# MichSchli/RelationPrediction

Measured on AMD Instinct MI355X. Metric: processed edges/sec (R-GCN forward+backward), FB15k-237 gcn_block, higher is better.
Workload: dtype f32 (dense contractions: fp32 operands split exactly into 3 bf16, 6 of 9 partial products on the bf16 matrix cores, fp32 accumulation; error vs float64 equal to the fp32 MFMA's); 1 GPU; fb237_block; entities=14541, relations=237, dim=500, layers=2, kind=block, num_blocks_or_bases=100, graph_edges=15000, norm_mode=intended (1/deg of the edge's own row; SURVEY H1, DESIGN section 10), parallelism=single GPU

## Files before the change

### include/rgcn_devtools.h

```cpp
#ifndef RGCN_DEVTOOLS_H_
#define RGCN_DEVTOOLS_H_

#include "rgcn.h"

#ifdef __cplusplus
extern "C" {
#endif
#if defined(__GNUC__)
#pragma GCC visibility push(default)
#endif

rgcn_status rgcn_debug_gemm(rgcn_ctx* ctx, int32_t trans_a, int32_t trans_b, int32_t M, int32_t N,
                            int32_t K, int32_t split_k, const float* a_host, const float* b_host,
                            float* c_host);

rgcn_status rgcn_debug_gemm_time(rgcn_ctx* ctx, int32_t trans_a, int32_t trans_b, int32_t M, int32_t N,
                                 int32_t K, int32_t split_k, int32_t iters, const float* a_host,
                                 const float* b_host, float* avg_ms);

rgcn_status rgcn_debug_gemm_presplit(rgcn_ctx* ctx, int32_t trans_b, int32_t M, int32_t N, int32_t K, int32_t iters,
                                     const float* a_host, const float* b_host, float* c_host, float* avg_ms);

rgcn_status rgcn_debug_xcd_map(rgcn_ctx* ctx, int32_t n_blocks, int32_t* out_host);

#if defined(__GNUC__)
#pragma GCC visibility pop
#endif
#ifdef __cplusplus
}
#endif
#endif
```

### relationprediction_amd/_native.py

```python
from __future__ import annotations

import ctypes as C
import os

import numpy as np

_HERE = os.path.dirname(os.path.abspath(__file__))
LIB_PATH = os.path.join(_HERE, "lib", "librgcn.so")

ABI_VERSION = 1
KIND_BLOCK, KIND_BASIS = 0, 1
NORM_INTENDED, NORM_TF_AS_EXECUTED, NORM_NONE, NORM_LOCAL = 0, 1, 2, 3
BUF_EXCHANGE, BUF_SELF, BUF_DSELF_EXCHANGE, BUF_INDEG, BUF_OUTDEG, BUF_ROWPTR, BUF_NORM_EXCHANGE, \
    BUF_DBASIS_EXCHANGE, BUF_PERM_VERTEX, BUF_PERM_RELATION, BUF_RANK_ENERGIES, BUF_MSG_NORM = range(12)

KINDS = {"block": KIND_BLOCK, "basis": KIND_BASIS}
NORMS = {"intended": NORM_INTENDED, "tf_as_executed": NORM_TF_AS_EXECUTED, "none": NORM_NONE, "local": NORM_LOCAL}

INPUT_EMBEDDING, INPUT_ONEHOT = 0, 1
INPUT_MODES = {"embedding": INPUT_EMBEDDING, "onehot": INPUT_ONEHOT}


def norm_mode_value(norm_mode):
    if isinstance(norm_mode, str):
        if norm_mode not in NORMS:
            raise ValueError("IncidenceNormalization / norm_mode must be one of %s, not %r"
                             % (", ".join(sorted(NORMS, key=NORMS.get)), norm_mode))
        return NORMS[norm_mode]
    return int(norm_mode)


class RgcnError(RuntimeError):
    def __init__(self, status, message):
        super().__init__("librgcn status %d: %s" % (status, message))
        self.status = status


class RgcnConfig(C.Structure):
    _fields_ = [
        ("abi_version", C.c_int32), ("device", C.c_int32), ("num_entities", C.c_int32),
        ("num_relations", C.c_int32), ("dim", C.c_int32), ("num_layers", C.c_int32),
        ("kind", C.c_int32), ("num_bases", C.c_int32), ("keep_prob", C.c_float),
        ("norm_mode", C.c_int32), ("max_edges", C.c_int64), ("rank", C.c_int32),
        ("world", C.c_int32), ("input_mode", C.c_int32),
    ]


_lib = None

_P = C.c_void_p
_SIGS = {
    "rgcn_abi_version": (C.c_int32, []),
    "rgcn_create": (C.c_int32, [C.POINTER(RgcnConfig), C.POINTER(_P)]),
    "rgcn_destroy": (C.c_int32, [_P]),
    "rgcn_last_error": (C.c_char_p, [_P]),
    "rgcn_sync": (C.c_int32, [_P]),
    "rgcn_param_count": (C.c_int32, [_P]),
    "rgcn_param_info": (C.c_int32, [_P, C.c_int32, C.c_char_p, C.c_int32, C.POINTER(C.c_int64), C.POINTER(C.c_int32)]),
    "rgcn_set_param": (C.c_int32, [_P, C.c_int32, _P, C.c_int64]),
    "rgcn_get_param": (C.c_int32, [_P, C.c_int32, _P, C.c_int64]),
    "rgcn_get_grad": (C.c_int32, [_P, C.c_int32, _P, C.c_int64]),
    "rgcn_set_graph": (C.c_int32, [_P, _P, C.c_int64]),
    "rgcn_set_graph_device": (C.c_int32, [_P, _P, C.c_int64]),
    "rgcn_forward": (C.c_int32, [_P, C.c_int32, C.c_uint64, _P]),
    "rgcn_get_codes": (C.c_int32, [_P, _P, C.c_int64]),
    "rgcn_get_activation": (C.c_int32, [_P, C.c_int32, _P, C.c_int64]),
    "rgcn_get_dropout_mask": (C.c_int32, [_P, C.c_int32, _P, C.c_int64]),
    "rgcn_codes_device": (_P, [_P]),
    "rgcn_backward": (C.c_int32, [_P, _P, C.c_int64]),
    "rgcn_backward_device": (C.c_int32, [_P, _P]),
    "rgcn_step_device": (C.c_int32, [_P, _P, C.c_int64, C.c_int32, C.c_uint64, _P]),
    "rgcn_decoder_reserve": (C.c_int32, [_P, C.c_int64]),
    "rgcn_decoder_loss_backward_device": (C.c_int32, [_P, _P, _P, C.c_int64, C.c_float]),
    "rgcn_dcodes_device": (_P, [_P]),
    "rgcn_get_loss": (C.c_int32, [_P, C.POINTER(C.c_double)]),
    "rgcn_optimizer_config": (C.c_int32, [_P, C.c_float, C.c_float, C.c_float, C.c_float, C.c_float]),
    "rgcn_sampler_create": (C.c_int32, [_P, C.c_int64, C.c_int32, C.POINTER(_P)]),
    "rgcn_sampler_destroy": (None, [_P]),
    "rgcn_sampler_edge_neighborhood": (C.c_int32, [_P, C.c_int64, C.c_uint64, _P]),
    "rgcn_neighborhood_reserve": (C.c_int32, [_P, _P, C.c_int64]),
    "rgcn_sample_neighborhood_device": (C.c_int32, [_P, C.c_int64, C.c_uint64, _P, C.c_int32]),
    "rgcn_capture_begin": (C.c_int32, [_P]),
    "rgcn_capture_end": (C.c_int32, [_P, C.POINTER(C.c_int32)]),
    "rgcn_graph_launch": (C.c_int32, [_P, C.c_int32]),
    "rgcn_graph_destroy": (C.c_int32, [_P, C.c_int32]),
    "rgcn_negative_sample_device": (C.c_int32, [_P, _P, C.c_int64, C.c_int32, C.c_uint64, _P, _P]),
    "rgcn_rank_reserve": (C.c_int32, [_P, C.c_int64]),
    "rgcn_rank_device": (C.c_int32, [_P, _P, C.c_int64, C.c_int32, _P, _P, _P, _P]),
    "rgcn_topk_device": (C.c_int32, [_P, _P, C.c_int64, C.c_int32, C.c_int32, _P, _P, _P, _P]),
    "rgcn_optimizer_step": (C.c_int32, [_P]),
    "rgcn_optimizer_norm_partial": (C.c_int32, [_P]),
    "rgcn_optimizer_apply": (C.c_int32, [_P]),
    "rgcn_train_step_device": (C.c_int32, [_P, _P, C.c_int64, _P, _P, C.c_int64, C.c_uint64, C.c_float]),
    "rgcn_prefetch_graph_device": (C.c_int32, [_P, _P, C.c_int64]),
    "rgcn_prefetch_graph_dropout_device": (C.c_int32, [_P, _P, C.c_int64, C.c_int64, C.c_uint64]),
    "rgcn_set_graph_dropout_device": (C.c_int32, [_P, _P, C.c_int64, C.c_int64, C.c_uint64, _P]),
    "rgcn_get_graph_edges": (C.c_int32, [_P, _P, C.c_int64]),
    "rgcn_train_step_minibatch_device": (C.c_int32, [_P, _P, C.c_int64, C.c_int64, C.c_uint64, C.c_int32, C.c_uint64,
                                                     _P, _P, C.c_uint64, C.c_float]),
    "rgcn_set_relation_owner": (C.c_int32, [_P, _P, C.c_int32]),
    "rgcn_comm_unique_id": (C.c_int32, [_P]),
    "rgcn_comm_init": (C.c_int32, [_P, _P]),
    "rgcn_comm_allreduce_sum": (C.c_int32, [_P, _P, C.c_int64]),
    "rgcn_forward_begin": (C.c_int32, [_P, C.c_int32, C.c_uint64, _P]),
    "rgcn_forward_layer_partial": (C.c_int32, [_P, C.c_int32]),
    "rgcn_forward_layer_finish": (C.c_int32, [_P, C.c_int32]),
    "rgcn_backward_begin": (C.c_int32, [_P, _P]),
    "rgcn_backward_layer_partial": (C.c_int32, [_P, C.c_int32]),
    "rgcn_backward_layer_finish": (C.c_int32, [_P, C.c_int32]),
    "rgcn_backward_end": (C.c_int32, [_P]),
    "rgcn_read_buffer": (C.c_int32, [_P, C.c_int32, _P, C.c_int64]),
    "rgcn_write_buffer": (C.c_int32, [_P, C.c_int32, _P, C.c_int64]),
    "rgcn_device_alloc": (C.c_int32, [_P, C.c_int64, C.POINTER(_P)]),
    "rgcn_device_free": (C.c_int32, [_P, _P]),
    "rgcn_copy_to_device": (C.c_int32, [_P, _P, _P, C.c_int64]),
    "rgcn_copy_to_device_async": (C.c_int32, [_P, _P, _P, C.c_int64, C.c_int32]),
    "rgcn_copy_to_host": (C.c_int32, [_P, _P, _P, C.c_int64]),
    "rgcn_timer_start": (C.c_int32, [_P]),
    "rgcn_timer_stop": (C.c_int32, [_P, C.POINTER(C.c_float)]),
    "rgcn_set_overlap": (C.c_int32, [_P, C.c_int32]),
    "rgcn_set_gemm_mode": (C.c_int32, [_P, C.c_int32]),
    "rgcn_set_fusion": (C.c_int32, [_P, C.c_int32]),
    "rgcn_comm_info": (C.c_int32, [_P, C.POINTER(C.c_int32), C.POINTER(C.c_int32), C.POINTER(C.c_int32)]),
    "rgcn_device_info": (C.c_int32, [C.c_int32, C.POINTER(C.c_int32), C.POINTER(C.c_int64)]),
    "rgcn_profile_enable": (C.c_int32, [_P, C.c_int32]),
    "rgcn_profile_reset": (C.c_int32, [_P]),
    "rgcn_profile_count": (C.c_int32, [_P]),
    "rgcn_profile_get_compulsory": (C.c_int32, [_P, C.c_int32, C.POINTER(C.c_double)]),
    "rgcn_profile_get": (C.c_int32, [_P, C.c_int32, C.c_char_p, C.c_int32, C.POINTER(C.c_int64),
                                    C.POINTER(C.c_double), C.POINTER(C.c_double), C.POINTER(C.c_double)]),
}
_DEVTOOLS_SIGS = {
    "rgcn_debug_gemm": (C.c_int32, [_P, C.c_int32, C.c_int32, C.c_int32, C.c_int32, C.c_int32, C.c_int32, _P, _P, _P]),
    "rgcn_debug_xcd_map": (C.c_int32, [_P, C.c_int32, _P]),
    "rgcn_debug_gemm_presplit": (C.c_int32, [_P, C.c_int32, C.c_int32, C.c_int32, C.c_int32, C.c_int32, _P, _P, _P,
                                             C.POINTER(C.c_float)]),
    "rgcn_debug_gemm_time": (C.c_int32, [_P, C.c_int32, C.c_int32, C.c_int32, C.c_int32, C.c_int32, C.c_int32,
                                         C.c_int32, _P, _P, C.POINTER(C.c_float)]),
}
_lib_devtools = None


def exported_symbols():
    return sorted(_SIGS)


def exported_devtools_symbols():
    return sorted(_DEVTOOLS_SIGS)


def load_library(path=None, devtools=False):
    global _lib, _lib_devtools
    if devtools:
        if _lib_devtools is None or path is not None:
            p = path or os.path.join(os.path.dirname(LIB_PATH), "librgcn_devtools.so")
            if not os.path.exists(p):
                raise ImportError("%s not found: python -m relationprediction_amd.build makes it" % p)
            lib = C.CDLL(p, mode=C.RTLD_LOCAL)
            for name, (res, args) in list(_SIGS.items()) + list(_DEVTOOLS_SIGS.items()):
                fn = getattr(lib, name)
                fn.restype = res
                fn.argtypes = args
            if path is not None:
                return lib
            _lib_devtools = lib
        return _lib_devtools
    if _lib is not None and path is None:
        return _lib
    if path is None and os.environ.get("RGCN_LIBRARY") == "devtools":
        _lib = load_library(devtools=True)
        return _lib
    p = path or LIB_PATH
    if not os.path.exists(p):
        raise ImportError(
            "%s not found: build the HIP library first (python -m relationprediction_amd.build, or "
            "__graft_entry__.build()).  There is no CPU fallback." % p)
    lib = C.CDLL(p, mode=C.RTLD_GLOBAL)
    for name, (res, args) in _SIGS.items():
        fn = getattr(lib, name)
        fn.restype = res
        fn.argtypes = args
    if lib.rgcn_abi_version() != ABI_VERSION:
        raise ImportError("librgcn.so ABI version %d != binding %d" % (lib.rgcn_abi_version(), ABI_VERSION))
    if path is None:
        _lib = lib
    return lib


def _ptr(a):
    return a.ctypes.data_as(C.c_void_p)


class DeviceBuffer:

    def __init__(self, engine, nbytes):
        self.engine = engine
        self.nbytes = int(nbytes)
        p = C.c_void_p()
        engine._check(engine.lib.rgcn_device_alloc(engine.ctx, self.nbytes, C.byref(p)))
        self.ptr = p

    def upload(self, arr):
        arr = np.ascontiguousarray(arr)
        assert arr.nbytes == self.nbytes, (arr.nbytes, self.nbytes)
        self.engine._check(self.engine.lib.rgcn_copy_to_device(self.engine.ctx, self.ptr, _ptr(arr), arr.nbytes))
        return self

    def download(self, dtype, shape):
        out = np.empty(shape, dtype=dtype)
        assert out.nbytes <= self.nbytes
        self.engine._check(self.engine.lib.rgcn_copy_to_host(self.engine.ctx, _ptr(out), self.ptr, out.nbytes))
        return out

    def free(self):
        if self.ptr is not None and self.engine.ctx is not None:
            self.engine.lib.rgcn_device_free(self.engine.ctx, self.ptr)
        self.ptr = None


class NeighborhoodSampler:

    def __init__(self, triples, num_entities):
        self.lib = load_library()
        t = np.ascontiguousarray(triples, dtype=np.int32).reshape(-1, 3)
        self.n = len(t)
        h = C.c_void_p()
        st = self.lib.rgcn_sampler_create(_ptr(t), self.n, int(num_entities), C.byref(h))
        if st != 0:
            raise RgcnError(st, "rgcn_sampler_create (ids out of range or empty graph)")
        self.handle = h

    def sample(self, sample_size, seed):
        out = np.empty(int(sample_size), dtype=np.int32)
        st = self.lib.rgcn_sampler_edge_neighborhood(self.handle, int(sample_size), C.c_uint64(int(seed)), _ptr(out))
        if st != 0:
            raise RgcnError(st, "rgcn_sampler_edge_neighborhood (sample_size %d of %d edges)" % (sample_size, self.n))
        return out

    def close(self):
        if getattr(self, "handle", None) is not None:
            self.lib.rgcn_sampler_destroy(self.handle)
            self.handle = None

    __del__ = close


class Engine:

    def __init__(self, num_entities, num_relations, dim, num_layers, kind, num_bases, keep_prob=0.8,
                 norm_mode="intended", max_edges=0, device=0, rank=0, world=1, devtools=False, input_mode="embedding"):
        self.lib = load_library(devtools=devtools)
        self.ctx = None
        cfg = RgcnConfig()
        cfg.abi_version = ABI_VERSION
        cfg.device = int(device)
        cfg.num_entities = int(num_entities)
        cfg.num_relations = int(num_relations)
        cfg.dim = int(dim)
        cfg.num_layers = int(num_layers)
        cfg.kind = KINDS[kind] if isinstance(kind, str) else int(kind)
        cfg.num_bases = int(num_bases)
        cfg.keep_prob = float(keep_prob)
        cfg.norm_mode = norm_mode_value(norm_mode)
        cfg.max_edges = int(max_edges)
        cfg.rank = int(rank)
        cfg.world = int(world)
        cfg.input_mode = INPUT_MODES[input_mode] if isinstance(input_mode, str) else int(input_mode)
        self.cfg = cfg
        ctx = C.c_void_p()
        st = self.lib.rgcn_create(C.byref(cfg), C.byref(ctx))
        if st != 0:
            raise RgcnError(st, (self.lib.rgcn_last_error(None) or b"").decode())
        self.ctx = ctx
        self.V, self.R, self.d, self.L = cfg.num_entities, cfg.num_relations, cfg.dim, cfg.num_layers
        self.max_edges = int(cfg.max_edges)
        self.param_names, self.param_shapes = [], []
        for i in range(self.lib.rgcn_param_count(self.ctx)):
            name = C.create_string_buffer(64)
            shape = (C.c_int64 * 4)()
            nd = C.c_int32()
            self._check(self.lib.rgcn_param_info(self.ctx, i, name, 64, shape, C.byref(nd)))
            self.param_names.append(name.value.decode())
            self.param_shapes.append(tuple(int(shape[k]) for k in range(nd.value)))

    def _check(self, st):
        if st != 0:
            raise RgcnError(st, (self.lib.rgcn_last_error(self.ctx) or b"").decode())

    def close(self):
        if self.ctx is not None:
            if getattr(self, "_rank_buf", None) is not None:
                self._rank_buf.free()
                self._rank_buf = None
            self.lib.rgcn_destroy(self.ctx)
            self.ctx = None

    def __del__(self):
        try:
            self.close()
        except Exception:
            pass

    def __enter__(self):
        return self

    def __exit__(self, *a):
        self.close()

    def sync(self):
        self._check(self.lib.rgcn_sync(self.ctx))

    def _index(self, key):
        return key if isinstance(key, int) else self.param_names.index(key)

    def set_param(self, key, value):
        i = self._index(key)
        a = np.ascontiguousarray(value, dtype=np.float32)
        if tuple(a.shape) != self.param_shapes[i]:
            raise ValueError("%s: shape %s != %s" % (self.param_names[i], a.shape, self.param_shapes[i]))
        self._check(self.lib.rgcn_set_param(self.ctx, i, _ptr(a), a.size))

    def set_params(self, params):
        for n in self.param_names:
            self.set_param(n, params[n])

    def get_param(self, key):
        i = self._index(key)
        out = np.empty(self.param_shapes[i], dtype=np.float32)
        self._check(self.lib.rgcn_get_param(self.ctx, i, _ptr(out), out.size))
        return out

    def get_grad(self, key):
        i = self._index(key)
        out = np.empty(self.param_shapes[i], dtype=np.float32)
        self._check(self.lib.rgcn_get_grad(self.ctx, i, _ptr(out), out.size))
        return out

    def get_grads(self):
        return {n: self.get_grad(n) for n in self.param_names}

    def get_params(self):
        return {n: self.get_param(n) for n in self.param_names}

    def set_graph(self, triples):
        t = np.asarray(triples)
        if t.size == 0:
            t = np.zeros((0, 3), dtype=np.int32)
        if t.ndim != 2 or t.shape[1] != 3:
            raise ValueError("graph_edges must be [E,3]")
        if t.dtype != np.int32:
            if t.size and (t.min() < -2 ** 31 or t.max() >= 2 ** 31):
                raise ValueError("ids do not fit int32")
            t = t.astype(np.int32)
        t = np.ascontiguousarray(t)
        self._check(self.lib.rgcn_set_graph(self.ctx, _ptr(t), t.shape[0]))
        self.num_edges = int(t.shape[0])

    def set_graph_device(self, dev_buffer, num_edges):
        self._check(self.lib.rgcn_set_graph_device(self.ctx, dev_buffer.ptr, int(num_edges)))
        self.num_edges = int(num_edges)

    def set_graph_dropout_device(self, batch_buffer, num_edges, keep, seed=0, keep_mask=None):
        self._check(self.lib.rgcn_set_graph_dropout_device(self.ctx, batch_buffer.ptr, int(num_edges), int(keep),
                                                           C.c_uint64(seed), keep_mask.ptr if keep_mask else None))
        self.num_edges = int(keep)

    def graph_edges(self):
        out = np.empty((self.num_edges, 3), dtype=np.int32)
        self._check(self.lib.rgcn_get_graph_edges(self.ctx, _ptr(out), self.num_edges))
        return out

    def prefetch_graph_dropout_device(self, batch_buffer, num_edges, keep, seed):
        self._check(self.lib.rgcn_prefetch_graph_dropout_device(self.ctx, batch_buffer.ptr, int(num_edges), int(keep),
                                                                C.c_uint64(seed)))

    def train_step_minibatch_device(self, batch_buffer, num_edges, keep, edge_seed, rate, negative_seed, x_dev, y_dev,
                                    seed=0, reg_param=0.01):
        self._check(self.lib.rgcn_train_step_minibatch_device(
            self.ctx, batch_buffer.ptr, int(num_edges), int(keep), C.c_uint64(edge_seed), int(rate),
            C.c_uint64(negative_seed), x_dev.ptr, y_dev.ptr, C.c_uint64(seed), C.c_float(reg_param)))
        self.num_edges = int(keep)

    def set_relation_owner(self, owner):
        o = np.ascontiguousarray(owner, dtype=np.int32)
        self._check(self.lib.rgcn_set_relation_owner(self.ctx, _ptr(o), o.size))

    def _masks(self, masks):
        if masks is None:
            return None, None
        m = np.ascontiguousarray(np.stack([np.asarray(x) for x in masks]).astype(np.uint8))
        if m.shape != (self.L, self.V, self.d):
            raise ValueError("dropout masks must be [L,V,d]")
        return m, _ptr(m)

    def forward(self, train=True, seed=0, masks=None):
        m, p = self._masks(masks)
        self._check(self.lib.rgcn_forward(self.ctx, 1 if train else 0, C.c_uint64(seed), p))

    def codes(self):
        return self.activation(self.L)

    def activation(self, layer):
        out = np.empty((self.V, self.d), dtype=np.float32)
        self._check(self.lib.rgcn_get_activation(self.ctx, int(layer), _ptr(out), out.size))
        return out

    def dropout_mask(self, layer):
        out = np.empty((self.V, self.d), dtype=np.uint8)
        self._check(self.lib.rgcn_get_dropout_mask(self.ctx, int(layer), _ptr(out), out.size))
        return out

    def backward(self, dcodes):
        g = np.ascontiguousarray(dcodes, dtype=np.float32)
        if g.shape != (self.V, self.d):
            raise ValueError("dcodes must be [V,d]")
        self._check(self.lib.rgcn_backward(self.ctx, _ptr(g), g.size))

    def backward_device(self, dev_buffer):
        self._check(self.lib.rgcn_backward_device(self.ctx, dev_buffer.ptr))

    def step_device(self, triples_dev, num_edges, dcodes_dev, train=True, seed=0):
        self._check(self.lib.rgcn_step_device(self.ctx, triples_dev.ptr, int(num_edges), 1 if train else 0,
                                              C.c_uint64(seed), dcodes_dev.ptr))
        self.num_edges = int(num_edges)

    def decoder_reserve(self, max_triples):
        self._check(self.lib.rgcn_decoder_reserve(self.ctx, int(max_triples)))

    def decoder_loss_backward_device(self, x_dev, y_dev, num_triples, reg_param):
        self._check(self.lib.rgcn_decoder_loss_backward_device(self.ctx, x_dev.ptr, y_dev.ptr, int(num_triples),
                                                               C.c_float(reg_param)))

    def backward_from_decoder(self):
        self._check(self.lib.rgcn_backward_device(self.ctx, self.lib.rgcn_dcodes_device(self.ctx)))

    def dcodes(self):
        out = np.empty((self.V, self.d), dtype=np.float32)
        self._check(self.lib.rgcn_copy_to_host(self.ctx, _ptr(out), self.lib.rgcn_dcodes_device(self.ctx), out.nbytes))
        return out

    def loss(self):
        v = C.c_double()
        self._check(self.lib.rgcn_get_loss(self.ctx, C.byref(v)))
        return float(v.value)

    def capture_begin(self):
        self._check(self.lib.rgcn_capture_begin(self.ctx))

    def capture_end(self):
        gid = C.c_int32(-1)
        self._check(self.lib.rgcn_capture_end(self.ctx, C.byref(gid)))
        return int(gid.value)

    def graph_launch(self, graph_id):
        self._check(self.lib.rgcn_graph_launch(self.ctx, int(graph_id)))

    def graph_destroy(self, graph_id):
        self._check(self.lib.rgcn_graph_destroy(self.ctx, int(graph_id)))

    def neighborhood_reserve(self, train_triples):
        t = np.ascontiguousarray(train_triples, dtype=np.int32).reshape(-1, 3)
        self._check(self.lib.rgcn_neighborhood_reserve(self.ctx, _ptr(t), len(t)))
        self._nbr_edges = len(t)

    def sample_neighborhood_device(self, sample_size, seed, batch_dev, on_prefetch_stream=False):
        self._check(self.lib.rgcn_sample_neighborhood_device(self.ctx, int(sample_size), C.c_uint64(int(seed)),
                                                             batch_dev.ptr, 1 if on_prefetch_stream else 0))

    def negative_sample_device(self, batch_dev, n, rate, seed, x_dev, y_dev):
        self._check(self.lib.rgcn_negative_sample_device(self.ctx, batch_dev.ptr, int(n), int(rate), C.c_uint64(int(seed)),
                                                         x_dev.ptr, y_dev.ptr))

    def rank_reserve(self, max_queries):
        self._check(self.lib.rgcn_rank_reserve(self.ctx, int(max_queries)))
        self._rank_reserved = max(getattr(self, "_rank_reserved", 0), int(max_queries))

    def ranks(self, triples, predict_object, filter_ptr, filter_idx):
        x = np.ascontiguousarray(triples, dtype=np.int32).reshape(-1, 3)
        n = len(x)
        if n == 0:
            return np.zeros(0, np.int32), np.zeros(0, np.int32)
        fp = np.ascontiguousarray(filter_ptr, dtype=np.int64)
        fi = np.ascontiguousarray(filter_idx, dtype=np.int32)
        assert fp.shape == (n + 1,) and fp[-1] == len(fi)
        nnz = max(len(fi), 1)
        off_x, off_fi = 8 * (n + 1), 8 * (n + 1) + 12 * n
        off_out = (off_fi + 4 * nnz + 7) // 8 * 8
        total = off_out + 8 * n
        if getattr(self, "_rank_buf", None) is None or self._rank_buf.nbytes < total:
            if getattr(self, "_rank_buf", None) is not None:
                self._rank_buf.free()
            self._rank_buf = DeviceBuffer(self, max(total, 1 << 20))
        base = self._rank_buf.ptr.value if hasattr(self._rank_buf.ptr, "value") else int(self._rank_buf.ptr)
        head = np.empty(off_fi, dtype=np.uint8)
        head[:off_x] = fp.view(np.uint8)
        head[off_x:] = x.reshape(-1).view(np.uint8)
        self._check(self.lib.rgcn_copy_to_device_async(self.ctx, C.c_void_p(base), _ptr(head), off_fi, 0))
        fb = fi.view(np.uint8)
        for lo in range(0, len(fb), 1 << 20):
            part = fb[lo:lo + (1 << 20)]
            self._check(self.lib.rgcn_copy_to_device_async(self.ctx, C.c_void_p(base + off_fi + lo), _ptr(part), len(part), 0))
        self._check(self.lib.rgcn_rank_device(self.ctx, C.c_void_p(base + off_x), n, 1 if predict_object else 0,
                                              C.c_void_p(base), C.c_void_p(base + off_fi), C.c_void_p(base + off_out),
                                              C.c_void_p(base + off_out + 4 * n)))
        out = np.empty(2 * n, dtype=np.int32)
        self._check(self.lib.rgcn_copy_to_host(self.ctx, _ptr(out), C.c_void_p(base + off_out), 8 * n))
        return out[:n].copy(), out[n:].copy()

    def topk(self, queries, predict_object, k, exclude_ptr=None, exclude_idx=None):
        x = np.ascontiguousarray(queries, dtype=np.int32).reshape(-1, 3)
        n, k = len(x), int(k)
        if (exclude_ptr is None) != (exclude_idx is None):
            raise ValueError("exclude_ptr and exclude_idx come together")
        if n == 0:
            return np.zeros((0, max(k, 0)), np.int32), np.zeros((0, max(k, 0)), np.float32)
        has = exclude_ptr is not None
        fp = np.ascontiguousarray(exclude_ptr if has else np.zeros(n + 1), dtype=np.int64)
        fi = np.ascontiguousarray(exclude_idx if has else np.zeros(0), dtype=np.int32)
        assert fp.shape == (n + 1,) and fp[-1] == len(fi)
        nnz = max(len(fi), 1)
        off_x, off_fi = 8 * (n + 1), 8 * (n + 1) + 12 * n
        off_out = (off_fi + 4 * nnz + 7) // 8 * 8
        room = min(max(k, 0), 1024)
        total = off_out + 8 * n * room
        if getattr(self, "_rank_buf", None) is None or self._rank_buf.nbytes < total:
            if getattr(self, "_rank_buf", None) is not None:
                self._rank_buf.free()
            self._rank_buf = DeviceBuffer(self, max(total, 1 << 20))
        base = self._rank_buf.ptr.value if hasattr(self._rank_buf.ptr, "value") else int(self._rank_buf.ptr)
        head = np.empty(off_fi, dtype=np.uint8)
        head[:off_x] = fp.view(np.uint8)
        head[off_x:] = x.reshape(-1).view(np.uint8)
        for lo in range(0, off_fi, 1 << 20):
            part = head[lo:lo + (1 << 20)]
            self._check(self.lib.rgcn_copy_to_device_async(self.ctx, C.c_void_p(base + lo), _ptr(part), len(part), 0))
        fb = fi.view(np.uint8)
        for lo in range(0, len(fb), 1 << 20):
            part = fb[lo:lo + (1 << 20)]
            self._check(self.lib.rgcn_copy_to_device_async(self.ctx, C.c_void_p(base + off_fi + lo), _ptr(part), len(part), 0))
        self._check(self.lib.rgcn_topk_device(self.ctx, C.c_void_p(base + off_x), n, 1 if predict_object else 0, k,
                                              C.c_void_p(base) if has else None,
                                              C.c_void_p(base + off_fi) if has else None, C.c_void_p(base + off_out),
                                              C.c_void_p(base + off_out + 4 * n * k)))
        out = np.empty(2 * n * k, dtype=np.int32)
        self._check(self.lib.rgcn_copy_to_host(self.ctx, _ptr(out), C.c_void_p(base + off_out), 8 * n * k))
        return out[:n * k].reshape(n, k).copy(), out[n * k:].view(np.float32).reshape(n, k).copy()

    def optimizer_config(self, lr=0.01, beta1=0.9, beta2=0.999, eps=1e-8, max_grad_norm=1.0):
        self._check(self.lib.rgcn_optimizer_config(self.ctx, lr, beta1, beta2, eps, max_grad_norm))

    def optimizer_step(self):
        self._check(self.lib.rgcn_optimizer_step(self.ctx))

    def optimizer_norm_partial(self):
        self._check(self.lib.rgcn_optimizer_norm_partial(self.ctx))

    def optimizer_apply(self):
        self._check(self.lib.rgcn_optimizer_apply(self.ctx))

    def train_step_device(self, triples_dev, num_edges, x_dev, y_dev, num_triples, seed=0, reg_param=0.01):
        self._check(self.lib.rgcn_train_step_device(self.ctx, triples_dev.ptr, int(num_edges), x_dev.ptr, y_dev.ptr,
                                                    int(num_triples), C.c_uint64(seed), C.c_float(reg_param)))
        self.num_edges = int(num_edges)

    def prefetch_graph_device(self, triples_dev, num_edges):
        self._check(self.lib.rgcn_prefetch_graph_device(self.ctx, triples_dev.ptr, int(num_edges)))

    def forward_begin(self, train=True, seed=0, masks=None):
        m, p = self._masks(masks)
        self._check(self.lib.rgcn_forward_begin(self.ctx, 1 if train else 0, C.c_uint64(seed), p))

    def forward_layer_partial(self, l):
        self._check(self.lib.rgcn_forward_layer_partial(self.ctx, l))

    def forward_layer_finish(self, l):
        self._check(self.lib.rgcn_forward_layer_finish(self.ctx, l))

    def backward_begin(self, dcodes_dev=None):
        ptr = self.lib.rgcn_dcodes_device(self.ctx) if dcodes_dev is None else dcodes_dev.ptr
        self._check(self.lib.rgcn_backward_begin(self.ctx, ptr))

    def backward_layer_partial(self, l):
        self._check(self.lib.rgcn_backward_layer_partial(self.ctx, l))

    def backward_layer_finish(self, l):
        self._check(self.lib.rgcn_backward_layer_finish(self.ctx, l))

    def backward_end(self):
        self._check(self.lib.rgcn_backward_end(self.ctx))

    def read_buffer(self, which):
        if which in (BUF_INDEG, BUF_OUTDEG):
            out = np.empty(self.V, dtype=np.int32)
        elif which == BUF_ROWPTR:
            out = np.empty(self.V + 1, dtype=np.int32)
        elif which in (BUF_PERM_VERTEX, BUF_PERM_RELATION):
            out = np.empty(2 * self.num_edges, dtype=np.int32)
        elif which == BUF_MSG_NORM:
            out = np.empty(2 * self.num_edges, dtype=np.float32)
        elif which == BUF_RANK_ENERGIES:
            out = np.empty((getattr(self, "_rank_reserved", 0), self.V), dtype=np.float32)
        elif which == BUF_DSELF_EXCHANGE:
            out = np.empty((self.d, self.d), dtype=np.float32)
        elif which == BUF_NORM_EXCHANGE:
            out = np.empty(1, dtype=np.float32)
        elif which == BUF_DBASIS_EXCHANGE:
            out = np.empty((2, int(self.cfg.num_bases), self.d, self.d), dtype=np.float32)
        else:
            out = np.empty((self.V, self.d), dtype=np.float32)
        self._check(self.lib.rgcn_read_buffer(self.ctx, which, _ptr(out), out.nbytes))
        return out

    def write_buffer(self, which, arr):
        a = np.ascontiguousarray(arr, dtype=np.float32)
        self._check(self.lib.rgcn_write_buffer(self.ctx, which, _ptr(a), a.nbytes))

    @staticmethod
    def comm_unique_id():
        lib = load_library()
        buf = (C.c_uint8 * 128)()
        st = lib.rgcn_comm_unique_id(buf)
        if st != 0:
            raise RgcnError(st, (lib.rgcn_last_error(None) or b"").decode())
        return bytes(buf)

    @staticmethod
    def device_info(device=0):
        lib = load_library()
        n, pci = C.c_int32(0), C.c_int64(-1)
        st = lib.rgcn_device_info(int(device), C.byref(n), C.byref(pci))
        if st != 0:
            raise RgcnError(st, (lib.rgcn_last_error(None) or b"").decode())
        return n.value, pci.value

    def comm_init(self, unique_id):
        buf = (C.c_uint8 * 128).from_buffer_copy(bytes(unique_id))
        self._check(self.lib.rgcn_comm_init(self.ctx, buf))

    def comm_info(self):
        n, r, dev = C.c_int32(-1), C.c_int32(-1), C.c_int32(-1)
        self._check(self.lib.rgcn_comm_info(self.ctx, C.byref(n), C.byref(r), C.byref(dev)))
        return n.value, r.value, dev.value

    def comm_allreduce_sum(self, dev_buffer, count):
        self._check(self.lib.rgcn_comm_allreduce_sum(self.ctx, dev_buffer.ptr, int(count)))

    def alloc(self, nbytes):
        return DeviceBuffer(self, nbytes)

    def copy_to_device(self, buf, arr):
        arr = np.ascontiguousarray(arr)
        assert arr.nbytes <= buf.nbytes
        self._check(self.lib.rgcn_copy_to_device(self.ctx, buf.ptr, _ptr(arr), arr.nbytes))

    def copy_to_device_async(self, buf, arr, on_prefetch_stream=False):
        arr = np.ascontiguousarray(arr)
        assert arr.nbytes <= buf.nbytes
        self._check(self.lib.rgcn_copy_to_device_async(self.ctx, buf.ptr, _ptr(arr), arr.nbytes,
                                                       1 if on_prefetch_stream else 0))

    def to_device(self, arr):
        arr = np.ascontiguousarray(arr)
        return DeviceBuffer(self, arr.nbytes).upload(arr)

    def timer_start(self):
        self._check(self.lib.rgcn_timer_start(self.ctx))

    def timer_stop(self):
        ms = C.c_float()
        self._check(self.lib.rgcn_timer_stop(self.ctx, C.byref(ms)))
        return float(ms.value)

    def set_overlap(self, on=True):
        self._check(self.lib.rgcn_set_overlap(self.ctx, 1 if on else 0))

    def set_fusion(self, mode):
        self._check(self.lib.rgcn_set_fusion(self.ctx, int(mode)))

    def set_gemm_mode(self, mode):
        self._check(self.lib.rgcn_set_gemm_mode(self.ctx, int(mode)))

    def profile_enable(self, on=True):
        self._check(self.lib.rgcn_profile_enable(self.ctx, 1 if on else 0))

    def profile_reset(self):
        self._check(self.lib.rgcn_profile_reset(self.ctx))

    def profile(self):
        out = []
        n = self.lib.rgcn_profile_count(self.ctx)
        for i in range(n):
            name = C.create_string_buffer(64)
            calls = C.c_int64()
            ms, by, fl = C.c_double(), C.c_double(), C.c_double()
            self._check(self.lib.rgcn_profile_get(self.ctx, i, name, 64, C.byref(calls), C.byref(ms),
                                                  C.byref(by), C.byref(fl)))
            cb = C.c_double()
            self._check(self.lib.rgcn_profile_get_compulsory(self.ctx, i, C.byref(cb)))
            out.append({"name": name.value.decode(), "calls": calls.value, "total_ms": ms.value,
                        "alg_bytes": by.value, "alg_flops": fl.value, "compulsory_bytes": cb.value})
        return out

    def debug_gemm_presplit(self, a, b, trans_b=False, iters=0):
        a = np.ascontiguousarray(a, dtype=np.float32)
        b = np.ascontiguousarray(b, dtype=np.float32)
        M, K = a.shape
        N = b.shape[0] if trans_b else b.shape[1]
        out = np.empty((M, N), dtype=np.float32)
        ms = C.c_float()
        self._check(self.lib.rgcn_debug_gemm_presplit(self.ctx, int(trans_b), M, N, K, int(iters), _ptr(a), _ptr(b),
                                                      _ptr(out), C.byref(ms)))
        return (out, float(ms.value)) if iters else out

    def debug_xcd_map(self, n_blocks):
        out = np.zeros(int(n_blocks), dtype=np.int32)
        self._check(self.lib.rgcn_debug_xcd_map(self.ctx, int(n_blocks), _ptr(out)))
        return out

    def debug_gemm_time(self, a, b, trans_a=False, trans_b=False, split_k=0, iters=20):
        a = np.ascontiguousarray(a, dtype=np.float32)
        b = np.ascontiguousarray(b, dtype=np.float32)
        K, M = (a.shape if trans_a else a.shape[::-1])
        N = b.shape[0] if trans_b else b.shape[1]
        ms = C.c_float()
        self._check(self.lib.rgcn_debug_gemm_time(self.ctx, int(trans_a), int(trans_b), M, N, K, int(split_k),
                                                  int(iters), _ptr(a), _ptr(b), C.byref(ms)))
        return float(ms.value)

    def debug_gemm(self, a, b, trans_a=False, trans_b=False, split_k=0):
        a = np.ascontiguousarray(a, dtype=np.float32)
        b = np.ascontiguousarray(b, dtype=np.float32)
        K, M = (a.shape if trans_a else a.shape[::-1])
        N = b.shape[0] if trans_b else b.shape[1]
        assert (b.shape[1] if trans_b else b.shape[0]) == K
        out = np.empty((M, N), dtype=np.float32)
        self._check(self.lib.rgcn_debug_gemm(self.ctx, int(trans_a), int(trans_b), M, N, K, int(split_k),
                                             _ptr(a), _ptr(b), _ptr(out)))
        return out
```

### relationprediction_amd/build.py

```python
from __future__ import annotations

import hashlib
import os
import shutil
import subprocess
import sys
from concurrent.futures import ThreadPoolExecutor

HERE = os.path.dirname(os.path.abspath(__file__))
ROOT = os.path.dirname(HERE)
CSRC = os.path.join(HERE, "csrc")
OBJDIR = os.path.join(ROOT, "build", "obj")
LIBDIR = os.path.join(HERE, "lib")
LIB = os.path.join(LIBDIR, "librgcn.so")
LIB_DEVTOOLS = os.path.join(LIBDIR, "librgcn_devtools.so")
ARCH = "gfx950"
SOURCES = ["rgcn_api.hip", "rgcn_schedule.hip", "rgcn_devtools.hip", "graph_prep.hip", "csr_sort.hip", "gemm_f32.hip", "gemm_bf16x3.hip", "gemm_bf16x3_w8.hip", "block_msgs.hip", "block_rows.hip", "basis.hip", "basis_onehot.hip",
           "elementwise.hip", "decoder.hip", "optimizer.hip", "ranking.hip", "sampler.hip", "neighborhood.hip", "comm.hip"]
HEADERS = [os.path.join(CSRC, "rgcn_internal.h"), os.path.join(CSRC, "rgcn_api_internal.h"), os.path.join(CSRC, "gemm_split.h"), os.path.join(ROOT, "include", "rgcn.h"),
           os.path.join(ROOT, "include", "rgcn_devtools.h")]
DEVTOOLS_SOURCES = ["rgcn_api.hip", "rgcn_devtools.hip", "comm.hip", "decoder.hip", "gemm_bf16x3.hip", "gemm_bf16x3_w8.hip"]
NO_PACKED_FP32 = ["-Xclang", "-target-feature", "-Xclang", "-packed-fp32-ops"]
FLAGS = ["--offload-arch=" + ARCH, "-O3", "-std=c++17", "-fPIC", "-fvisibility=hidden", "-Wall",
         "-Wno-unused-function"] + NO_PACKED_FP32


def _hipcc():
    for cand in (shutil.which("hipcc"), "/opt/rocm/bin/hipcc"):
        if cand and os.path.exists(cand):
            return cand
    raise RuntimeError("hipcc not found: the R-GCN HIP library cannot be built")


def _digest(paths):
    h = hashlib.sha256()
    h.update(" ".join(FLAGS).encode())
    for p in paths:
        with open(p, "rb") as f:
            h.update(f.read())
    return h.hexdigest()


def _llvm_objdump():
    for cand in ("/opt/rocm/lib/llvm/bin/llvm-objdump", shutil.which("llvm-objdump")):
        if cand and os.path.exists(cand):
            return cand
    return None


def check_no_packed_fp32(lib=None):
    import glob
    import re
    import tempfile
    lib = lib or LIB
    objdump = _llvm_objdump()
    if objdump is None:
        raise RuntimeError("llvm-objdump not found: cannot verify the library is free of packed-FP32 ops")
    with tempfile.TemporaryDirectory() as tmp:
        copy = os.path.join(tmp, "lib.so")
        shutil.copy(lib, copy)
        subprocess.run([objdump, "--offloading", copy], capture_output=True, text=True, cwd=tmp, check=True)
        bad = []
        objs = glob.glob(copy + ".*amdgcn*")
        if not objs:
            raise RuntimeError("no device code objects found in " + lib)
        for co in objs:
            r = subprocess.run([objdump, "-d", co], capture_output=True, text=True, check=True)
            bad += re.findall(r"v_pk_(?:fma|mul|add)_f32", r.stdout)
        if bad:
            raise RuntimeError("librgcn.so contains %d packed-FP32 instructions (%s): they are unsafe beside the "
                               "bf16-split GEMM" % (len(bad), ", ".join(sorted(set(bad)))))
    return True


def build(force=False, verbose=False):
    os.makedirs(OBJDIR, exist_ok=True)
    os.makedirs(LIBDIR, exist_ok=True)
    hipcc = _hipcc()
    jobs = []
    for src in SOURCES + [d + "@devtools" for d in DEVTOOLS_SOURCES]:
        dev = src.endswith("@devtools")
        src = src.replace("@devtools", "")
        sp = os.path.join(CSRC, src)
        obj = os.path.join(OBJDIR, src.replace(".hip", ".devtools.o" if dev else ".o"))
        stamp = obj + ".sha"
        dig = _digest([sp] + HEADERS) + ("+devtools" if dev else "")
        fresh = (not force and os.path.exists(obj) and os.path.exists(stamp)
                 and open(stamp).read() == dig)
        jobs.append((sp, obj, stamp, dig, fresh, dev))

    def compile_one(job):
        sp, obj, stamp, dig, fresh, dev = job
        if fresh:
            return None
        cmd = [hipcc] + FLAGS + (["-DRGCN_DEVTOOLS"] if dev else []) + ["-c", sp, "-o", obj]
        r = subprocess.run(cmd, capture_output=True, text=True)
        if r.returncode != 0:
            raise RuntimeError("hipcc failed for %s:\n%s" % (sp, r.stderr[-4000:]))
        with open(stamp, "w") as f:
            f.write(dig)
        return r.stderr if verbose else None

    with ThreadPoolExecutor(max_workers=min(8, len(jobs))) as ex:
        outs = list(ex.map(compile_one, jobs))
    for o in outs:
        if o:
            sys.stderr.write(o)
    product = [j for j in jobs if not j[5]]
    devobj = {os.path.basename(j[0]): j[1] for j in jobs if j[5]}
    stale = any(not j[4] for j in jobs)
    for lib, objs in ((LIB, [j[1] for j in product]),
                      (LIB_DEVTOOLS, [devobj.get(os.path.basename(j[0]), j[1]) for j in product])):
        if force or stale or not os.path.exists(lib):
            vs = os.path.join(OBJDIR, "exports.map")
            with open(vs, "w") as f:
                f.write("{ global: rgcn_*; local: *; };\n")
            cmd = [hipcc, "--offload-arch=" + ARCH, "-shared", "-fPIC", "-Wl,--version-script=" + vs, "-o", lib] + objs + ["-ldl"]
            r = subprocess.run(cmd, capture_output=True, text=True)
            if r.returncode != 0:
                raise RuntimeError("link failed:\n" + r.stderr[-4000:])
            check_no_packed_fp32(lib)
    return LIB


def build_test_collective(force=False, device_side=False):
    root = os.path.dirname(os.path.dirname(os.path.abspath(__file__)))
    name = "ipc_collective" if device_side else "shm_collective"
    src = os.path.join(root, "tests", "collective_double", name + ".hip")
    outdir = os.path.join(root, "tests", "collective_double", "_build")
    out = os.path.join(outdir, "lib%s.so" % name.replace("_", ""))
    stamp = out + ".sha"
    dig = _digest([src])
    if not force and os.path.exists(out) and os.path.exists(stamp) and open(stamp).read() == dig:
        return out
    os.makedirs(outdir, exist_ok=True)
    r = subprocess.run([_hipcc(), "--offload-arch=" + ARCH, "-O2", "-std=c++17", "-fPIC", "-shared", src, "-o", out,
                        "-lrt"], capture_output=True, text=True)
    if r.returncode != 0:
        raise RuntimeError("hipcc failed for %s:\n%s" % (src, r.stderr[-4000:]))
    with open(stamp, "w") as f:
        f.write(dig)
    return out


if __name__ == "__main__":
    print(build(force="--force" in sys.argv, verbose="--verbose" in sys.argv))
```

### relationprediction_amd/csrc/gemm_bf16x3.hip

```cpp
#include <cstdlib>

#include "gemm_split.h"

namespace rgcn {

using namespace gx;

namespace {

template <bool VEC>
__device__ __forceinline__ void load_kc(const float* __restrict__ X, const float* __restrict__ zeros,
                                        int ld, int rows, int row0, int k0, int kend, f32x4 (&r)[2]) {
#pragma unroll
  for (int p = 0; p < 2; ++p) {
    const int f = threadIdx.x + NTH * p;
    const int row = row0 + (f >> 2), k = k0 + (f & 3) * 4;
    const size_t off = (size_t)row * ld + k;
    if constexpr (VEC) {
      const float* src = (row < rows && k < kend) ? X + off : zeros;
      r[p] = *reinterpret_cast<const f32x4*>(src);
    } else {
      float e[4];
#pragma unroll
      for (int q = 0; q < 4; ++q) {
        const float* src = (row < rows && k + q < kend) ? X + off + q : zeros;
        e[q] = *src;
      }
      r[p] = f32x4{e[0], e[1], e[2], e[3]};
    }
  }
}
template <bool VEC>
__device__ __forceinline__ void load_rc(const float* __restrict__ X, const float* __restrict__ zeros,
                                        int ld, int rows, int row0, int k0, int kend, f32x4 (&r)[2]) {
  const int kp = threadIdx.x >> 5, rg = threadIdx.x & 31;
#pragma unroll
  for (int q = 0; q < 2; ++q) {
    const int k = k0 + 2 * kp + q, row = row0 + 4 * rg;
    const size_t off = (size_t)k * ld + row;
    if constexpr (VEC) {
      const float* src = (k < kend && row < rows) ? X + off : zeros;
      r[q] = *reinterpret_cast<const f32x4*>(src);
    } else {
      float e[4];
#pragma unroll
      for (int i = 0; i < 4; ++i) {
        const float* src = (k < kend && row + i < rows) ? X + off + i : zeros;
        e[i] = *src;
      }
      r[q] = f32x4{e[0], e[1], e[2], e[3]};
    }
  }
}

struct SplitRegs {
  u32x4 w;
};
template <bool KC, int PLANE, int C>
__device__ __forceinline__ void split_chunk(f32x4 (&r)[2], SplitRegs& st, uint32_t* __restrict__ lds,
                                            uint32_t negmask) {
  if constexpr (KC) {
    constexpr int q = C / 6, c = C % 6;
    const int f = threadIdx.x + NTH * q;
    uint32_t* dst = lds + (f >> 2) * KC_LD + (f & 3) * 2;
    f32x4& v = r[q];
    if constexpr (c == 0 || c == 2) st.w[0] = split_level<0, 1>(v, v, c == 0 ? negmask : 0u);
    if constexpr (c == 1 || c == 3) {
      st.w[1] = split_level<2, 3>(v, v, c == 1 ? negmask : 0u);
      *reinterpret_cast<uint2*>(dst + (c / 2) * PLANE) = make_uint2(st.w[0], st.w[1]);
    }
    if constexpr (c == 4)
      *reinterpret_cast<uint2*>(dst + 2 * PLANE) = make_uint2(split_last(v[0], v[1]), split_last(v[2], v[3]));
  } else {
    const int kp = threadIdx.x >> 5, rg = threadIdx.x & 31;
    uint32_t* dst = lds + kp * RC_LD + 4 * rg;
    f32x4& e = r[0];
    f32x4& o = r[1];
    if constexpr (C < 8) {
      constexpr int i = C % 4;
      st.w[i] = split_level<i, i>(e, o, C < 4 ? negmask : 0u);
      if constexpr (i == 3) *reinterpret_cast<u32x4*>(dst + (C / 4) * PLANE) = st.w;
    }
    if constexpr (C == 8) { st.w[0] = split_last(e[0], o[0]); st.w[1] = split_last(e[1], o[1]); }
    if constexpr (C == 9) {
      st.w[2] = split_last(e[2], o[2]); st.w[3] = split_last(e[3], o[3]);
      *reinterpret_cast<u32x4*>(dst + 2 * PLANE) = st.w;
    }
  }
}
template <bool KC, int PLANE, int C0, int C1>
__device__ __forceinline__ void split_chunks(f32x4 (&r)[2], SplitRegs& st, uint32_t* __restrict__ lds,
                                             uint32_t negmask = 0u) {
  if constexpr (C0 < C1) {
    split_chunk<KC, PLANE, C0>(r, st, lds, negmask);
    split_chunks<KC, PLANE, C0 + 1, C1>(r, st, lds, negmask);
  }
}

template <bool KC>
__device__ __forceinline__ bf16x8 load_frag(const uint32_t* __restrict__ plane, int row, int h) {
  u32x4 v;
  if constexpr (KC) {
    v = *reinterpret_cast<const u32x4*>(plane + row * KC_LD + 4 * h);
  } else {
    const uint32_t* p = plane + (4 * h) * RC_LD + row;
    v[0] = p[0]; v[1] = p[RC_LD]; v[2] = p[2 * RC_LD]; v[3] = p[3 * RC_LD];
  }
  return __builtin_bit_cast(bf16x8, v);
}

template <bool A_KC, bool B_KC, bool VEC, int TERMS, bool B_PRE = false>
__global__ void __launch_bounds__(NTH, 2) k_gemm_bf16x3(XArgs g) {
  constexpr int PA = A_KC ? KC_PLANE : RC_PLANE, PB = B_KC ? KC_PLANE : RC_PLANE;
  constexpr int TA = 3 * PA, TB = B_PRE ? 0 : 3 * PB;
  extern __shared__ __attribute__((aligned(16))) uint32_t lds[];

  int wg = blockIdx.x;
  const int total = g.tiles_m * g.tiles_n * g.splits;
  if (g.swizzle == 1) {
    const int xcd = wg & 7, idx = wg >> 3;
    const int q = total >> 3, r = total & 7;
    wg = (xcd < r ? xcd * (q + 1) : r * (q + 1) + (xcd - r) * q) + idx;
  }
  const int per_split = g.tiles_m * g.tiles_n;
  int z = wg / per_split;
  const int rem = wg - z * per_split;
  int m0 = (rem / g.tiles_n) * BM, n0 = (rem % g.tiles_n) * BN;
  if (g.swizzle == 2) {
    const int xcd = blockIdx.x & 7, idx = blockIdx.x >> 3;
    const int rp = (idx / g.tiles_n) * 8 + xcd;
    if (rp >= g.tiles_m) return;
    z = 0;
    m0 = rp * BM;
    n0 = (idx % g.tiles_n) * BN;
  }
  const int grp = blockIdx.y;
  int Mlim = g.M, Klim = g.K, kps = g.k_per_split;
  if (g.batch.limit != nullptr) {
    const int n = g.batch.limit[grp * g.batch.limit_stride];
    if (g.batch.limit_on_k) {
      Klim = min(Klim, max(n, 0));
      const int per = (Klim + g.splits - 1) / g.splits;
      kps = max(BK, ((per + BK - 1) / BK) * BK);
    } else {
      Mlim = min(Mlim, n);
      if (m0 >= Mlim) return;
    }
  }
  const float* const gA = g.A + (size_t)grp * g.batch.strideA;
  const float* const gB = g.B + (size_t)grp * g.batch.strideB;
  const int ks = z * kps;
  const int ke = max(ks, min(Klim, ks + kps));
  const int nkt = (ke - ks + BK - 1) / BK;

  const int lane = threadIdx.x & 63, wave = threadIdx.x >> 6;
  const int wm = (wave >> 1) * 64, wn = (wave & 1) * 64;
  const int li = lane & 31, h = lane >> 5;

  f32x16 acc[2][2];
#pragma unroll
  for (int i = 0; i < 2; ++i)
#pragma unroll
    for (int j = 0; j < 2; ++j)
#pragma unroll
      for (int r = 0; r < 16; ++r) acc[i][j][r] = 0.0f;

  f32x4 ra[2][2], rb[2][2];
  auto gload = [&](int k0, f32x4 (&xa)[2], f32x4 (&xb)[2]) {
    if constexpr (A_KC) load_kc<VEC>(gA, g.zeros, g.lda, Mlim, m0, k0, ke, xa);
    else load_rc<VEC>(gA, g.zeros, g.lda, Mlim, m0, k0, ke, xa);
    if constexpr (!B_PRE) {
      if constexpr (B_KC) load_kc<VEC>(gB, g.zeros, g.ldb, g.N, n0, k0, ke, xb);
      else load_rc<VEC>(gB, g.zeros, g.ldb, g.N, n0, k0, ke, xb);
    }
  };
  const float* wa[2];
  const float* wb[2];
  int ia[2] = {0, 0}, ib[2] = {0, 0};
  if constexpr (VEC) {
#pragma unroll
    for (int p = 0; p < 2; ++p) {
      if constexpr (A_KC) {
        const int f = threadIdx.x + NTH * p, row = m0 + (f >> 2);
        wa[p] = row < Mlim ? gA + (size_t)row * g.lda + ks + (f & 3) * 4 : g.zeros;
        ia[p] = row < Mlim ? BK : 0;
      } else {
        const int row = m0 + 4 * (threadIdx.x & 31), k = ks + 2 * (threadIdx.x >> 5) + p;
        wa[p] = row < Mlim ? gA + (size_t)k * g.lda + row : g.zeros;
        ia[p] = row < Mlim ? BK * g.lda : 0;
      }
      if constexpr (B_PRE) {
        wb[p] = g.zeros;
      } else if constexpr (B_KC) {
        const int f = threadIdx.x + NTH * p, row = n0 + (f >> 2);
        wb[p] = row < g.N ? gB + (size_t)row * g.ldb + ks + (f & 3) * 4 : g.zeros;
        ib[p] = row < g.N ? BK : 0;
      } else {
        const int row = n0 + 4 * (threadIdx.x & 31), k = ks + 2 * (threadIdx.x >> 5) + p;
        wb[p] = row < g.N ? gB + (size_t)k * g.ldb + row : g.zeros;
        ib[p] = row < g.N ? BK * g.ldb : 0;
      }
    }
#pragma unroll
    for (int p = 0; p < 2; ++p) { wa[p] += 2 * (size_t)ia[p]; wb[p] += 2 * (size_t)ib[p]; }
  }
  auto gwalk = [&](f32x4 (&xa)[2], f32x4 (&xb)[2]) {
#pragma unroll
    for (int p = 0; p < 2; ++p) {
      xa[p] = *reinterpret_cast<const f32x4*>(wa[p]);
      wa[p] += ia[p];
      if constexpr (!B_PRE) {
        xb[p] = *reinterpret_cast<const f32x4*>(wb[p]);
        wb[p] += ib[p];
      }
    }
  };
  auto sstore = [&](uint32_t* buf, f32x4 (&xa)[2], f32x4 (&xb)[2]) {
    SplitRegs st;
    split_chunks<A_KC, PA, 0, 12>(xa, st, buf);
    if constexpr (!B_PRE) split_chunks<B_KC, PB, 0, 12>(xb, st, buf + TA);
  };
  const int nkt_all = (g.K + BK - 1) / BK;
  const u32x4* const bq = B_PRE ? g.bfrag + (size_t)grp * g.batch.strideBfrag +
                                      ((size_t)((n0 + wn) >> 5) * 6 + h) * 32 + li
                                : nullptr;
  bf16x8 fbp[2][2][3];
  auto bfetch = [&](int kt_abs, bf16x8 (&f)[2][3]) {
    const u32x4* q = bq + (size_t)min(kt_abs, nkt_all - 1) * g.nt32 * 192;
#pragma unroll
    for (int j = 0; j < 2; ++j)
#pragma unroll
      for (int pl = 0; pl < 3; ++pl) f[j][pl] = __builtin_bit_cast(bf16x8, q[(j * 3 + pl) * 64]);
  };
  int flip[3] = {1 << 30, 1 << 30, 1 << 30};
  if (nkt >= 16) {
    flip[0] = max(2, (int)(0.173f * nkt + 0.5f) & ~1);
    flip[1] = (nkt / 2 + 1) & ~1;
    flip[2] = (int)(0.849f * nkt + 0.5f) & ~1;
  }
  auto sign_group = [&](int t) { return (t >= flip[0] ? 1 : 0) + (t >= flip[1] ? 1 : 0) + (t >= flip[2] ? 1 : 0); };
  auto negate_acc = [&]() {
#pragma unroll
    for (int i = 0; i < 2; ++i)
#pragma unroll
      for (int j = 0; j < 2; ++j)
#pragma unroll
        for (int r = 0; r < 16; ++r) acc[i][j][r] = 0.0f - acc[i][j][r];
  };
  auto step = [&](int kt, auto parity, auto walk) {
    constexpr int P = decltype(parity)::value;
    constexpr bool WALK = decltype(walk)::value;
    if (kt == flip[0] || kt == flip[1] || kt == flip[2]) negate_acc();
    const uint32_t negmask = (sign_group(kt + 1) & 1) ? 0x80000000u : 0u;
    if constexpr (WALK) gwalk(ra[P], rb[P]); else gload(ks + (kt + 2) * BK, ra[P], rb[P]);
    if constexpr (B_PRE) bfetch(kt + 1, fbp[1 - P]);
    const uint32_t* a_lds = lds + P * (TA + TB);
    const uint32_t* b_lds = a_lds + TA;
    uint32_t* nxt = lds + (1 - P) * (TA + TB);
    bf16x8 fa[2][3], fb[2][3];
#pragma unroll
    for (int i = 0; i < 2; ++i)
#pragma unroll
      for (int pl = 0; pl < 3; ++pl) fa[i][pl] = load_frag<A_KC>(a_lds + pl * PA, wm + 32 * i + li, h);
#pragma unroll
    for (int j = 0; j < 2; ++j)
#pragma unroll
      for (int pl = 0; pl < 3; ++pl) {
        if constexpr (B_PRE) fb[j][pl] = fbp[P][j][pl];
        else fb[j][pl] = load_frag<B_KC>(b_lds + pl * PB, wn + 32 * j + li, h);
      }
    __builtin_amdgcn_sched_barrier(0);
    constexpr int NP = 9;
    constexpr int pa_[NP] = {2, 2, 1, 2, 0, 1, 1, 0, 0};
    constexpr int pb_[NP] = {2, 1, 2, 0, 2, 1, 0, 1, 0};
    constexpr int NM = 4 * TERMS;
    constexpr int NCH = B_PRE ? 12 : 24;
    constexpr int PER = (NCH + NM - 1) / NM;
    SplitRegs st;
    auto weave = [&](auto mi) {
      constexpr int m = decltype(mi)::value;
      constexpr int t = NP - TERMS + m / 4, i = (m / 2) % 2, j = m % 2;
      acc[i][j] = __builtin_amdgcn_mfma_f32_32x32x16_bf16(fa[i][pa_[t]], fb[j][pb_[t]], acc[i][j], 0, 0, 0);
      constexpr int c0 = B_PRE ? (m % 2 == 0 ? m / 2 : 12) : (m * PER < 24 ? m * PER : 24);
      constexpr int c1 = B_PRE ? (m % 2 == 0 ? (m / 2 + 1 < 12 ? m / 2 + 1 : 12) : 12) : ((m + 1) * PER < 24 ? (m + 1) * PER : 24);
      split_chunks<A_KC, PA, (c0 < 12 ? c0 : 12), (c1 < 12 ? c1 : 12)>(ra[1 - P], st, nxt, negmask);
      if constexpr (!B_PRE)
        split_chunks<B_KC, PB, (c0 > 12 ? c0 - 12 : 0), (c1 > 12 ? c1 - 12 : 0)>(rb[1 - P], st, nxt + TA);
      __builtin_amdgcn_sched_barrier(0);
    };
    static_for<0, NM>(weave);
    lds_barrier();
  };

  if (nkt > 0) {
    gload(ks, ra[0], rb[0]);
    if constexpr (B_PRE) bfetch(0, fbp[0]);
    sstore(lds, ra[0], rb[0]);
    gload(ks + BK, ra[1], rb[1]);
  }
  lds_barrier();
  using I0 = std::integral_constant<int, 0>;
  using I1 = std::integral_constant<int, 1>;
  int kt = 0;
  if constexpr (VEC) {
    const int nwalk = ((ke - ks) / BK - 2) & ~1;
    for (; kt < nwalk; kt += 2) {
      step(kt, I0{}, std::true_type{});
      step(kt + 1, I1{}, std::true_type{});
    }
  }
  for (; kt < nkt; kt += 2) {
    step(kt, I0{}, std::false_type{});
    if (kt + 1 < nkt) step(kt + 1, I1{}, std::false_type{});
  }
  if (nkt > 0 && (sign_group(nkt - 1) & 1)) negate_acc();

  float* C = g.C + (size_t)grp * g.batch.strideC + (size_t)z * g.M * g.ldc;
  if (g.vecC) {
    float* stage = reinterpret_cast<float*>(lds);
#pragma unroll
    for (int pass = 0; pass < 2; ++pass) {
      if (wm == 64 * pass) {
#pragma unroll
        for (int i = 0; i < 2; ++i)
#pragma unroll
          for (int j = 0; j < 2; ++j)
#pragma unroll
            for (int r = 0; r < 16; ++r) {
              const int row = 32 * i + (r & 3) + 8 * (r >> 2) + 4 * h;
              stage[row * EPI_LD + wn + 32 * j + li] = acc[i][j][r];
            }
      }
      __syncthreads();
      constexpr int C4 = BN / 4;
#pragma unroll
      for (int q = 0; q < 64 * C4 / NTH; ++q) {
        const int f = threadIdx.x + NTH * q;
        const int row = f / C4, c4 = f % C4;
        const int grow = m0 + 64 * pass + row, gcol = n0 + 4 * c4;
        if (grow < Mlim && gcol < g.N) {
          const float4 v = *reinterpret_cast<const float4*>(stage + row * EPI_LD + 4 * c4);
          *reinterpret_cast<float4*>(C + (size_t)grow * g.ldc + gcol) = v;
        }
      }
      __syncthreads();
    }
    return;
  }
#pragma unroll
  for (int i = 0; i < 2; ++i)
#pragma unroll
    for (int j = 0; j < 2; ++j) {
      const int col = n0 + wn + 32 * j + li;
      if (col < g.N) {
#pragma unroll
        for (int r = 0; r < 16; ++r) {
          const int row = m0 + wm + 32 * i + (r & 3) + 8 * (r >> 2) + 4 * h;
          if (row < Mlim) C[(size_t)row * g.ldc + col] = acc[i][j][r];
        }
      }
    }
}

constexpr size_t lds_bytes(bool a_kc, bool b_kc, bool b_pre = false) {
  const size_t tiles = 2 * 3 * ((a_kc ? KC_PLANE : RC_PLANE) + (b_pre ? 0 : (b_kc ? KC_PLANE : RC_PLANE))) * 4;
  const size_t epi = 64 * EPI_LD * 4;
  return tiles > epi ? tiles : epi;
}

template <bool A_KC, bool B_KC, bool VEC, int TERMS, bool B_PRE = false>
hipError_t launch_one(rgcn_ctx* c, const XArgs& g) {
  constexpr size_t bytes = lds_bytes(A_KC, B_KC, B_PRE);
  auto kern = k_gemm_bf16x3<A_KC, B_KC, VEC, TERMS, B_PRE>;
  static uint64_t configured = 0;
  const hipError_t e = set_dynamic_lds(reinterpret_cast<const void*>(kern), (int)bytes, c->cfg.device, configured);
  if (e != hipSuccess) return e;
  const int gx = g.swizzle == 2 ? ((g.tiles_m + 7) / 8) * 8 * g.tiles_n : g.tiles_m * g.tiles_n * g.splits;
  hipLaunchKernelGGL(kern, dim3((unsigned)gx, (unsigned)g.batch.groups), dim3(NTH), bytes, c->stream, g);
  return hipGetLastError();
}

template <bool VEC, int TERMS>
hipError_t launch_form(rgcn_ctx* c, bool a_kc, bool b_kc, const XArgs& g) {
  if constexpr (VEC) {
    if (g.bfrag != nullptr && a_kc) return launch_one<true, true, true, TERMS, true>(c, g);
  }
  if (a_kc && !b_kc) return launch_one<true, false, VEC, TERMS>(c, g);
  if (a_kc && b_kc) return launch_one<true, true, VEC, TERMS>(c, g);
  return launch_one<false, false, VEC, TERMS>(c, g);
}

struct PresplitJobs {
  PresplitJob j[8];
};
__global__ void __launch_bounds__(256) k_presplit_b(PresplitJobs jobs) {
  const PresplitJob job = jobs.j[blockIdx.y];
  const int ktiles = (job.K + BK - 1) / BK, nt32 = bfrag_nt32(job.N);
  const int i = blockIdx.x * 256 + threadIdx.x;
  if (i >= ktiles * nt32 * 64) return;
  const float* __restrict__ B = job.B;
  const int li = i & 31, h = (i >> 5) & 1, nt = (i >> 6) % nt32, kt = (i >> 6) / nt32;
  const int n = 32 * nt + li, k0 = 16 * kt + 8 * h;
  f32x4 lo4 = {0.f, 0.f, 0.f, 0.f}, hi4 = {0.f, 0.f, 0.f, 0.f};
  if (n < job.N) {
#pragma unroll
    for (int q = 0; q < 8; ++q) {
      const int k = k0 + q;
      const float x = k < job.K ? (job.b_kc ? B[(size_t)n * job.ldb + k] : B[(size_t)k * job.ldb + n]) : 0.0f;
      if (q < 4) lo4[q] = x; else hi4[q - 4] = x;
    }
  }
  u32x4* dst = reinterpret_cast<u32x4*>(job.F) + ((size_t)(kt * nt32 + nt) * 6 + h) * 32 + li;
#pragma unroll
  for (int level = 0; level < 3; ++level) {
    u32x4 w;
    if (level < 2) {
      w[0] = split_level<0, 1>(lo4, lo4); w[1] = split_level<2, 3>(lo4, lo4);
      w[2] = split_level<0, 1>(hi4, hi4); w[3] = split_level<2, 3>(hi4, hi4);
    } else {
      w[0] = split_last(lo4[0], lo4[1]); w[1] = split_last(lo4[2], lo4[3]);
      w[2] = split_last(hi4[0], hi4[1]); w[3] = split_last(hi4[2], hi4[3]);
    }
    dst[level * 64] = w;
  }
}

}

size_t gemm_bfrag_words(int K, int N) {
  return (size_t)((K + BK - 1) / BK) * bfrag_nt32(N) * 192;
}

rgcn_status gemm_presplit_b(rgcn_ctx* c, const PresplitJob* jobs, int n) {
  for (int j0 = 0; j0 < n; j0 += 8) {
    PresplitJobs pj;
    int nj = 0, max_threads = 0;
    double bytes = 0;
    for (; nj < 8 && j0 + nj < n; ++nj) {
      pj.j[nj] = jobs[j0 + nj];
      const PresplitJob& q = pj.j[nj];
      const int threads = ((q.K + BK - 1) / BK) * bfrag_nt32(q.N) * 64;
      if (threads > max_threads) max_threads = threads;
      bytes += 4.0 * q.K * q.N + 16.0 * 3 * threads;
    }
    for (int k = nj; k < 8; ++k) pj.j[k] = pj.j[0];
    ProfScope ps(c, "gemm_presplit_b", bytes, 0);
    hipLaunchKernelGGL(k_presplit_b, dim3((unsigned)((max_threads + 255) / 256), (unsigned)nj), dim3(256), 0, c->stream, pj);
    RGCN_HIP(c, hipGetLastError());
  }
  return RGCN_OK;
}

hipError_t gemm_bf16x3_launch(rgcn_ctx* c, int terms, bool a_kc, bool b_kc, bool vec, int M, int N, int K,
                              const float* A, int lda, const float* B, int ldb, float* C, int ldc,
                              int k_per_split, int splits, int swizzle, int vecC, const GemmBatch* batch) {
  XArgs g;
  if (batch) g.batch = *batch;
  g.bfrag = (batch && batch->bfrag && splits == 1 && a_kc && vec) ? reinterpret_cast<const u32x4*>(batch->bfrag) : nullptr;
  g.A = A; g.B = B; g.C = C; g.zeros = c->zeros;
  g.M = M; g.N = N; g.K = K; g.lda = lda; g.ldb = ldb; g.ldc = ldc;
  g.k_per_split = k_per_split; g.splits = splits; g.swizzle = swizzle; g.vecC = vecC;
  g.tiles_m = (M + BM - 1) / BM;
  g.tiles_n = (N + BN - 1) / BN;
  g.nt32 = bfrag_nt32(N);
  const int w8 = knob("RGCN_GEMM_W8", 1);
  bool wide = g.batch.wide != 0;
  if (wide && g.batch.limit == nullptr) {
    const long t = (long)((M + 127) / 128) * ((N + 255) / 256) * g.batch.groups;
    wide = t <= 256 && t >= 160;
  }
  if (g.bfrag != nullptr && !g.batch.limit_on_k && (terms == 6 || terms == 9) && (w8 >= 2 || (w8 == 1 && wide)))
    return gemm_bf16x3_w8_launch(c, terms, M, N, K, A, lda, C, ldc, swizzle, vecC, g.batch);
  if (terms == 9) return vec ? launch_form<true, 9>(c, a_kc, b_kc, g) : launch_form<false, 9>(c, a_kc, b_kc, g);
  if (terms == 3) return vec ? launch_form<true, 3>(c, a_kc, b_kc, g) : launch_form<false, 3>(c, a_kc, b_kc, g);
  return vec ? launch_form<true, 6>(c, a_kc, b_kc, g) : launch_form<false, 6>(c, a_kc, b_kc, g);
}

}
```

### relationprediction_amd/csrc/gemm_bf16x3_w8.hip

```cpp
#include "gemm_split.h"

namespace rgcn {

using namespace gx;

namespace {

constexpr int WBM = 128, WBN = 256, WNTH = 512;
constexpr int A_HS = 2048 + 64;
constexpr int A_PL = 2 * A_HS;
constexpr int A_SZ = 12800;
constexpr int B_SZ = 24 * 1024;
constexpr int ST_SZ = A_SZ + B_SZ;
constexpr int W_LDS_BYTES = 4 * ST_SZ;
constexpr int WEPI_LD = WBN + 4;

__device__ __forceinline__ void aload(f32x4& dst, const float* p) {
  asm volatile("global_load_dwordx4 %0, %1, off" : "=v"(dst) : "v"(p) : "memory");
}
__device__ __forceinline__ void aload_s(f32x4& dst, uint32_t voff, const float* sbase) {
  asm volatile("global_load_dwordx4 %0, %1, %2" : "=v"(dst) : "v"(voff), "s"(sbase) : "memory");
}
template <int PIECE>
__device__ __forceinline__ void dma1(uint32_t voff, const u32x4* sbase, uint32_t lds_addr) {
  uint32_t keep;
  asm volatile(
      "s_mov_b32 %0, m0\n\t"
      "s_mov_b32 m0, %3\n\t"
      "s_nop 0\n\t"
      "global_load_lds_dwordx4 %1, %2 offset:%4\n\t"
      "s_mov_b32 m0, %0"
      : "=&s"(keep)
      : "v"(voff), "s"(sbase), "s"(lds_addr), "i"(PIECE * 1024)
      : "memory");
}

template <int TERMS>
__global__ void __launch_bounds__(WNTH, 2) __attribute__((amdgpu_num_vgpr(192))) k_gemm_w8(XArgs g) {
  extern __shared__ __attribute__((aligned(16))) uint32_t lds[];

  int wg = blockIdx.x;
  const int total = g.tiles_m * g.tiles_n;
  if (g.swizzle == 1) {
    const int xcd = wg & 7, idx = wg >> 3;
    const int q = total >> 3, r = total & 7;
    wg = (xcd < r ? xcd * (q + 1) : r * (q + 1) + (xcd - r) * q) + idx;
  }
  int m0 = (wg / g.tiles_n) * WBM, n0 = (wg % g.tiles_n) * WBN;
  if (g.swizzle == 2) {
    const int xcd = blockIdx.x & 7, idx = blockIdx.x >> 3;
    const int rp = (idx / g.tiles_n) * 8 + xcd;
    if (rp >= g.tiles_m) return;
    m0 = rp * WBM;
    n0 = (idx % g.tiles_n) * WBN;
  }
  const int grp = blockIdx.y;
  int Mlim = g.M;
  if (g.batch.limit != nullptr) {
    Mlim = min(Mlim, g.batch.limit[grp * g.batch.limit_stride]);
    if (m0 >= Mlim) return;
  }
  const float* const gA = g.A + (size_t)grp * g.batch.strideA;
  const int nkt = (g.K + BK - 1) / BK;
  const int nfull = g.K / BK;

  const int lane = threadIdx.x & 63;
  const int wave = __builtin_amdgcn_readfirstlane(threadIdx.x >> 6);
  const int wm = (wave >> 2) * 64, wn = (wave & 3) * 64;
  const int li = lane & 31, h = lane >> 5;
  const uint32_t lds0 = (uint32_t)(uintptr_t)lds;

  f32x16 acc[2][2];
#pragma unroll
  for (int i = 0; i < 2; ++i)
#pragma unroll
    for (int j = 0; j < 2; ++j)
#pragma unroll
      for (int r = 0; r < 16; ++r) acc[i][j][r] = 0.0f;

  const int arow = threadIdx.x >> 2, aq = threadIdx.x & 3;
  const float* sa = gA + (size_t)m0 * g.lda;
  const uint32_t a_off = ((uint32_t)min(arow, Mlim - 1 - m0) * (uint32_t)g.lda + 4u * aq) * 4u;
  const bool atail_ok = 4 * aq < (g.K & (BK - 1));
  f32x4 ra[4];
  const uint32_t a_wr = (aq >> 1) * A_HS + arow * 16 + (aq & 1) * 8;
  const u32x4* sb = g.bfrag + (size_t)grp * g.batch.strideBfrag + ((size_t)(n0 >> 5) + wave) * 192;
  const size_t sb_step = (size_t)g.nt32 * 192;
  const u32x4* const szero = reinterpret_cast<const u32x4*>(g.zeros);
  const uint32_t voff = lane * 16;
  const uint32_t b_wr = A_SZ + wave * 3072;
  const uint32_t a_rd = h * A_HS + (wm + li) * 16;
  const uint32_t b_rd = A_SZ + ((wave & 3) * 2) * 3072 + lane * 16;
  bf16x8 F[2][12];

  auto issue_part = [&](int s, auto slot, auto part) {
    constexpr int P = decltype(slot)::value;
    constexpr int Q = decltype(part)::value;
    const bool live = s < nkt;
    if constexpr (Q < 3) {
      dma1<Q>(voff, live ? sb : szero, lds0 + P * ST_SZ + b_wr);
      if constexpr (Q == 2) sb += sb_step;
    } else {
      if (s >= nfull) {
        const float* p = (live && atail_ok) ? reinterpret_cast<const float*>(reinterpret_cast<const char*>(sa) + a_off) : g.zeros;
        aload(ra[P], p);
      } else {
        aload_s(ra[P], a_off, sa);
      }
      sa += BK;
    }
  };
  auto issue = [&](int s, auto slot) {
    issue_part(s, slot, std::integral_constant<int, 0>{});
    issue_part(s, slot, std::integral_constant<int, 1>{});
    issue_part(s, slot, std::integral_constant<int, 2>{});
    issue_part(s, slot, std::integral_constant<int, 3>{});
  };
  int flip[3] = {1 << 30, 1 << 30, 1 << 30};
  if (nkt >= 16) {
    flip[0] = __builtin_amdgcn_readfirstlane(max(2, (int)(0.173f * nkt + 0.5f) & ~1));
    flip[1] = (nkt / 2 + 1) & ~1;
    flip[2] = __builtin_amdgcn_readfirstlane((int)(0.849f * nkt + 0.5f) & ~1);
  }
  auto sign_group = [&](int t) { return (t >= flip[0] ? 1 : 0) + (t >= flip[1] ? 1 : 0) + (t >= flip[2] ? 1 : 0); };
  auto negate_acc = [&]() {
#pragma unroll
    for (int i = 0; i < 2; ++i)
#pragma unroll
      for (int j = 0; j < 2; ++j)
#pragma unroll
        for (int r = 0; r < 16; ++r) acc[i][j][r] = 0.0f - acc[i][j][r];
  };
  uint32_t w0 = 0;
  auto split_piece = [&](auto piece, f32x4& v, uint32_t* dst, uint32_t negmask) {
    constexpr int c = decltype(piece)::value;
    if constexpr (c == 0 || c == 2) w0 = split_level<0, 1>(v, v, c == 0 ? negmask : 0u);
    if constexpr (c == 1 || c == 3) {
      const uint32_t w1 = split_level<2, 3>(v, v, c == 1 ? negmask : 0u);
      *reinterpret_cast<uint2*>(dst + (c / 2) * (A_PL / 4)) = make_uint2(w0, w1);
    }
    if constexpr (c == 4)
      *reinterpret_cast<uint2*>(dst + 2 * (A_PL / 4)) = make_uint2(split_last(v[0], v[1]), split_last(v[2], v[3]));
  };
  auto read_frag = [&](auto idx, const uint32_t* st, bf16x8 (&f)[12]) {
    constexpr int n = decltype(idx)::value;
    if constexpr (n < 6)
      f[n] = __builtin_bit_cast(bf16x8, *reinterpret_cast<const u32x4*>(st + (a_rd + (n / 3) * 512 + (n % 3) * A_PL) / 4));
    else
      f[n] = __builtin_bit_cast(bf16x8, *reinterpret_cast<const u32x4*>(st + (b_rd + ((n - 6) / 3) * 3072 + ((n - 6) % 3) * 1024) / 4));
  };

  constexpr int NP = 9;
  constexpr int pa_[NP] = {2, 2, 1, 2, 0, 1, 1, 0, 0};
  constexpr int pb_[NP] = {2, 1, 2, 0, 2, 1, 0, 1, 0};
  constexpr int NM = 4 * TERMS;
  constexpr int M_WAIT = NM / 2 - 2;
  auto step = [&](int t, auto slot, auto mf) {
    constexpr int P = decltype(slot)::value;
    constexpr bool MF = decltype(mf)::value;
    if (MF && (t == flip[0] || t == flip[1] || t == flip[2])) negate_acc();
    const uint32_t negmask = __builtin_amdgcn_readfirstlane((sign_group(t + 2) & 1) ? 0x80000000u : 0u);
    const uint32_t* st_rd = lds + ((P + 1) & 3) * (ST_SZ / 4);
    uint32_t* st_wr = lds + ((P + 2) & 3) * (ST_SZ / 4) + a_wr / 4;
    bf16x8(&fc)[12] = F[P & 1];
    bf16x8(&fn)[12] = F[(P + 1) & 1];
    f32x4& rs = ra[(P + 2) & 3];
    __builtin_amdgcn_sched_barrier(0);
    auto weave = [&](auto mi) {
      constexpr int m = decltype(mi)::value;
      if constexpr (MF) {
        constexpr int tt = NP - TERMS + m / 4, i = (m / 2) % 2, j = m % 2;
        acc[i][j] = __builtin_amdgcn_mfma_f32_32x32x16_bf16(fc[i * 3 + pa_[tt]], fc[6 + j * 3 + pb_[tt]], acc[i][j], 0, 0, 0);
      }
      if constexpr (m < 8 && m % 2 == 1) issue_part(t + 4, slot, std::integral_constant<int, m / 2>{});
      if constexpr (m < 12) read_frag(mi, st_rd, fn);
      if constexpr (m == M_WAIT) asm volatile("s_waitcnt vmcnt(8)" : "+v"(rs) : : "memory");
      if constexpr (m > M_WAIT && (m - M_WAIT) % 2 == 1 && (m - M_WAIT) / 2 < 5)
        split_piece(std::integral_constant<int, (m - M_WAIT) / 2>{}, rs, st_wr, negmask);
      __builtin_amdgcn_sched_barrier(0);
    };
    static_for<0, NM>(weave);
    lds_barrier();
  };

  using I0 = std::integral_constant<int, 0>;
  using I1 = std::integral_constant<int, 1>;
  using I2 = std::integral_constant<int, 2>;
  using I3 = std::integral_constant<int, 3>;
  issue(0, I0{});
  issue(1, I1{});
  step(-2, I2{}, std::false_type{});
  step(-1, I3{}, std::false_type{});
  int t = 0;
  for (; t + 4 <= nkt; t += 4) {
    step(t, I0{}, std::true_type{});
    step(t + 1, I1{}, std::true_type{});
    step(t + 2, I2{}, std::true_type{});
    step(t + 3, I3{}, std::true_type{});
  }
  if (t < nkt) step(t, I0{}, std::true_type{});
  if (t + 1 < nkt) step(t + 1, I1{}, std::true_type{});
  if (t + 2 < nkt) step(t + 2, I2{}, std::true_type{});
  if (nkt > 0 && (sign_group(nkt - 1) & 1)) negate_acc();
  asm volatile("s_waitcnt vmcnt(0)" : "+v"(ra[0]), "+v"(ra[1]), "+v"(ra[2]), "+v"(ra[3]) : : "memory");
  __syncthreads();

  float* C = g.C + (size_t)grp * g.batch.strideC;
  float* stage = reinterpret_cast<float*>(lds);
#pragma unroll
  for (int pass = 0; pass < 2; ++pass) {
#pragma unroll
    for (int j = 0; j < 2; ++j)
#pragma unroll
      for (int r = 0; r < 16; ++r) {
        const int row = (wm >> 1) + (r & 3) + 8 * (r >> 2) + 4 * h;
        stage[row * WEPI_LD + wn + 32 * j + li] = acc[pass][j][r];
      }
    __syncthreads();
    constexpr int C4 = WBN / 4;
#pragma unroll
    for (int q = 0; q < 64 * C4 / WNTH; ++q) {
      const int f = threadIdx.x + WNTH * q;
      const int row = f / C4, c4 = f % C4;
      const int grow = m0 + (row >> 5) * 64 + 32 * pass + (row & 31), gcol = n0 + 4 * c4;
      if (grow < Mlim && gcol < g.N) {
        const float4 v = *reinterpret_cast<const float4*>(stage + row * WEPI_LD + 4 * c4);
        if (g.vecC) {
          *reinterpret_cast<float4*>(C + (size_t)grow * g.ldc + gcol) = v;
        } else {
          float* o = C + (size_t)grow * g.ldc + gcol;
          o[0] = v.x;
          if (gcol + 1 < g.N) o[1] = v.y;
          if (gcol + 2 < g.N) o[2] = v.z;
          if (gcol + 3 < g.N) o[3] = v.w;
        }
      }
    }
    __syncthreads();
  }
}

template <int TERMS>
hipError_t launch_w8(rgcn_ctx* c, const XArgs& g) {
  auto kern = k_gemm_w8<TERMS>;
  static uint64_t configured = 0;
  const hipError_t e = set_dynamic_lds(reinterpret_cast<const void*>(kern), W_LDS_BYTES, c->cfg.device, configured);
  if (e != hipSuccess) return e;
  const int gx = g.swizzle == 2 ? ((g.tiles_m + 7) / 8) * 8 * g.tiles_n : g.tiles_m * g.tiles_n;
  hipLaunchKernelGGL(kern, dim3((unsigned)gx, (unsigned)g.batch.groups), dim3(WNTH), W_LDS_BYTES, c->stream, g);
  return hipGetLastError();
}

}

hipError_t gemm_bf16x3_w8_launch(rgcn_ctx* c, int terms, int M, int N, int K, const float* A, int lda, float* C, int ldc,
                                 int swizzle, int vecC, const GemmBatch& batch) {
  XArgs g;
  g.batch = batch;
  g.bfrag = reinterpret_cast<const u32x4*>(batch.bfrag);
  g.A = A; g.B = nullptr; g.C = C; g.zeros = c->zeros;
  g.M = M; g.N = N; g.K = K; g.lda = lda; g.ldb = 0; g.ldc = ldc;
  g.k_per_split = K; g.splits = 1; g.swizzle = swizzle; g.vecC = vecC;
  g.tiles_m = (M + WBM - 1) / WBM;
  g.tiles_n = (N + WBN - 1) / WBN;
  g.nt32 = bfrag_nt32(N);
  if (terms == 9) return launch_w8<9>(c, g);
  return launch_w8<6>(c, g);
}

}
```

### relationprediction_amd/csrc/gemm_f32.hip

```cpp
#include <cstdlib>

#include "rgcn_internal.h"

namespace rgcn {

namespace {

using f32x16 = __attribute__((ext_vector_type(16))) float;

struct GemmArgs {
  const float* A;
  const float* B;
  float* C;
  const float* zeros;
  int M, N, K;
  int lda, ldb, ldc;
  int k_per_split;
  int tiles_m, tiles_n, splits;
  int swizzle;
  int vecC;
  GemmBatch batch;
};

template <int BM_, int BN_, int BK_, int WGM_, int WGN_>
struct Cfg {
  static constexpr int BM = BM_, BN = BN_, BK = BK_, WGM = WGM_, WGN = WGN_;
  static constexpr int NT = 64 * WGM * WGN;
  static constexpr int TM = BM / WGM / 32, TN = BN / WGN / 32;
  static constexpr int LDK = BK + 4;
  static_assert(BM % (32 * WGM) == 0 && BN % (32 * WGN) == 0, "wave tiles are multiples of 32");
  static_assert(BK % 8 == 0, "BK multiple of 8");
  static_assert((BM * BK / 4) % NT == 0 && (BN * BK / 4) % NT == 0, "whole float4 passes");
};

template <bool KC, int ROWS, int BK, int NT, int P, bool VEC>
__device__ __forceinline__ void load_tile(const float* __restrict__ X, const float* __restrict__ zeros,
                                          int ld, int rows, int row0, int k0, int kend,
                                          float4 (&r)[P]) {
  const int t = threadIdx.x;
#pragma unroll
  for (int p = 0; p < P; ++p) {
    const int f = t + NT * p;
    int row, k;
    size_t off;
    if constexpr (KC) {
      constexpr int Q = BK / 4;
      row = row0 + f / Q;
      k = k0 + (f % Q) * 4;
      off = (size_t)row * ld + k;
    } else {
      constexpr int Q = ROWS / 4;
      k = k0 + f / Q;
      row = row0 + (f % Q) * 4;
      off = (size_t)k * ld + row;
    }
    if constexpr (VEC) {
      const bool ok = row < rows && k < kend;
      const float* src = ok ? X + off : zeros;
      r[p] = *reinterpret_cast<const float4*>(src);
    } else {
      float e[4];
#pragma unroll
      for (int q = 0; q < 4; ++q) {
        const bool ok = KC ? (row < rows && k + q < kend) : (k < kend && row + q < rows);
        const float* src = ok ? X + off + q : zeros;
        e[q] = *src;
      }
      r[p] = make_float4(e[0], e[1], e[2], e[3]);
    }
  }
}

template <bool KC, int ROWS, int BK, int NT, int P>
__device__ __forceinline__ void store_tile(float* __restrict__ lds, const float4 (&r)[P]) {
  const int t = threadIdx.x;
#pragma unroll
  for (int p = 0; p < P; ++p) {
    const int f = t + NT * p;
    int off;
    if constexpr (KC) off = (f / (BK / 4)) * (BK + 4) + (f % (BK / 4)) * 4;
    else off = (f / (ROWS / 4)) * ROWS + (f % (ROWS / 4)) * 4;
    *reinterpret_cast<float4*>(lds + off) = r[p];
  }
}

template <bool KC, int ROWS, int BK>
__device__ __forceinline__ void load_frag(const float* __restrict__ lds, int row, int kk, int h,
                                          float (&f)[4]) {
  if constexpr (KC) {
    const float4 v = *reinterpret_cast<const float4*>(lds + row * (BK + 4) + 8 * kk + 4 * h);
    f[0] = v.x; f[1] = v.y; f[2] = v.z; f[3] = v.w;
  } else {
    const float* p = lds + (8 * kk + 4 * h) * ROWS + row;
    f[0] = p[0]; f[1] = p[ROWS]; f[2] = p[2 * ROWS]; f[3] = p[3 * ROWS];
  }
}

template <bool A_KC, bool B_KC, bool VEC, class CF>
__global__ void __launch_bounds__(CF::NT) k_gemm_f32(GemmArgs g) {
  constexpr int BM = CF::BM, BN = CF::BN, BK = CF::BK, NT = CF::NT, TM = CF::TM, TN = CF::TN;
  constexpr int TA = A_KC ? BM * CF::LDK : BK * BM;
  constexpr int TB = B_KC ? BN * CF::LDK : BK * BN;
  constexpr int PA = BM * BK / 4 / NT, PB = BN * BK / 4 / NT;
  constexpr int EPI_LD = BN + 4;
  constexpr int EPI = 64 * EPI_LD;
  constexpr int LDS_FLOATS = 2 * (TA + TB) > EPI ? 2 * (TA + TB) : EPI;
  __shared__ __attribute__((aligned(16))) float lds[LDS_FLOATS];

  int wg = blockIdx.x;
  const int total = g.tiles_m * g.tiles_n * g.splits;
  if (g.swizzle == 1) {
    const int xcd = wg & 7, idx = wg >> 3;
    const int q = total >> 3, r = total & 7;
    wg = (xcd < r ? xcd * (q + 1) : r * (q + 1) + (xcd - r) * q) + idx;
  }
  const int per_split = g.tiles_m * g.tiles_n;
  int z = wg / per_split;
  const int rem = wg - z * per_split;
  int m0 = (rem / g.tiles_n) * BM, n0 = (rem % g.tiles_n) * BN;
  if (g.swizzle == 2) {
    const int xcd = blockIdx.x & 7, idx = blockIdx.x >> 3;
    const int rp = (idx / g.tiles_n) * 8 + xcd;
    if (rp >= g.tiles_m) return;
    z = 0;
    m0 = rp * BM;
    n0 = (idx % g.tiles_n) * BN;
  }
  const int grp = blockIdx.y;
  int Mlim = g.M, Klim = g.K, kps = g.k_per_split;
  if (g.batch.limit != nullptr) {
    const int n = g.batch.limit[grp * g.batch.limit_stride];
    if (g.batch.limit_on_k) {
      Klim = min(Klim, max(n, 0));
      const int per = (Klim + g.splits - 1) / g.splits;
      kps = max(BK, ((per + BK - 1) / BK) * BK);
    } else {
      Mlim = min(Mlim, n);
      if (m0 >= Mlim) return;
    }
  }
  const float* const gA = g.A + (size_t)grp * g.batch.strideA;
  const float* const gB = g.B + (size_t)grp * g.batch.strideB;
  const int ks = z * kps;
  const int ke = max(ks, min(Klim, ks + kps));
  const int nkt = (ke - ks + BK - 1) / BK;

  const int lane = threadIdx.x & 63, wave = threadIdx.x >> 6;
  const int wm = (wave / CF::WGN) * (TM * 32), wn = (wave % CF::WGN) * (TN * 32);
  const int li = lane & 31, h = lane >> 5;

  f32x16 acc[TM][TN];
#pragma unroll
  for (int i = 0; i < TM; ++i)
#pragma unroll
    for (int j = 0; j < TN; ++j)
#pragma unroll
      for (int r = 0; r < 16; ++r) acc[i][j][r] = 0.0f;

  float4 ra[PA], rb[PB];
  if (nkt > 0) {
    load_tile<A_KC, BM, BK, NT, PA, VEC>(gA, g.zeros, g.lda, Mlim, m0, ks, ke, ra);
    load_tile<B_KC, BN, BK, NT, PB, VEC>(gB, g.zeros, g.ldb, g.N, n0, ks, ke, rb);
    store_tile<A_KC, BM, BK, NT, PA>(lds, ra);
    store_tile<B_KC, BN, BK, NT, PB>(lds + TA, rb);
  }
  __syncthreads();

  for (int kt = 0; kt < nkt; ++kt) {
    const int cur = kt & 1;
    const bool more = kt + 1 < nkt;
    if (more) {
      load_tile<A_KC, BM, BK, NT, PA, VEC>(gA, g.zeros, g.lda, Mlim, m0, ks + (kt + 1) * BK, ke, ra);
      load_tile<B_KC, BN, BK, NT, PB, VEC>(gB, g.zeros, g.ldb, g.N, n0, ks + (kt + 1) * BK, ke, rb);
    }
    const float* a_lds = lds + cur * (TA + TB);
    const float* b_lds = a_lds + TA;
#pragma unroll
    for (int kk = 0; kk < BK / 8; ++kk) {
      float fa[TM][4], fb[TN][4];
#pragma unroll
      for (int i = 0; i < TM; ++i) load_frag<A_KC, BM, BK>(a_lds, wm + 32 * i + li, kk, h, fa[i]);
#pragma unroll
      for (int j = 0; j < TN; ++j) load_frag<B_KC, BN, BK>(b_lds, wn + 32 * j + li, kk, h, fb[j]);
#pragma unroll
      for (int t = 0; t < 4; ++t)
#pragma unroll
        for (int i = 0; i < TM; ++i)
#pragma unroll
          for (int j = 0; j < TN; ++j)
            acc[i][j] = __builtin_amdgcn_mfma_f32_32x32x2f32(fa[i][t], fb[j][t], acc[i][j], 0, 0, 0);
    }
    if (more) {
      store_tile<A_KC, BM, BK, NT, PA>(lds + (cur ^ 1) * (TA + TB), ra);
      store_tile<B_KC, BN, BK, NT, PB>(lds + (cur ^ 1) * (TA + TB) + TA, rb);
    }
    __syncthreads();
  }
  float* C = g.C + (size_t)grp * g.batch.strideC + (size_t)z * g.M * g.ldc;
  if (g.vecC) {
#pragma unroll
    for (int pass = 0; pass < BM / 64; ++pass) {
      if (wm / 64 == pass) {
#pragma unroll
        for (int i = 0; i < TM; ++i)
#pragma unroll
          for (int j = 0; j < TN; ++j)
#pragma unroll
            for (int r = 0; r < 16; ++r) {
              const int row = (wm % 64) + 32 * i + (r & 3) + 8 * (r >> 2) + 4 * h;
              lds[row * EPI_LD + wn + 32 * j + li] = acc[i][j][r];
            }
      }
      __syncthreads();
      constexpr int C4 = BN / 4;
#pragma unroll
      for (int q = 0; q < 64 * C4 / NT; ++q) {
        const int f = threadIdx.x + NT * q;
        const int row = f / C4, c4 = f % C4;
        const int grow = m0 + 64 * pass + row, gcol = n0 + 4 * c4;
        if (grow < Mlim && gcol < g.N) {
          const float4 v = *reinterpret_cast<const float4*>(lds + row * EPI_LD + 4 * c4);
          *reinterpret_cast<float4*>(C + (size_t)grow * g.ldc + gcol) = v;
        }
      }
      __syncthreads();
    }
    return;
  }
#pragma unroll
  for (int i = 0; i < TM; ++i)
#pragma unroll
    for (int j = 0; j < TN; ++j) {
      const int col = n0 + wn + 32 * j + li;
      if (col < g.N) {
#pragma unroll
        for (int r = 0; r < 16; ++r) {
          const int row = m0 + wm + 32 * i + (r & 3) + 8 * (r >> 2) + 4 * h;
          if (row < Mlim) C[(size_t)row * g.ldc + col] = acc[i][j][r];
        }
      }
    }
}

template <int VEC>
__global__ void k_splitk_reduce(const float* __restrict__ slab, float* __restrict__ C, int M, int N,
                                int ldc, int splits, size_t group_stride_c) {
  const int64_t i = ((int64_t)blockIdx.x * blockDim.x + threadIdx.x) * VEC;
  const int64_t mn = (int64_t)M * N;
  if (i >= mn) return;
  slab += (size_t)blockIdx.y * splits * mn;
  C += (size_t)blockIdx.y * group_stride_c;
  float acc[VEC];
#pragma unroll
  for (int k = 0; k < VEC; ++k) acc[k] = 0.0f;
  int s = 0;
  for (; s + 8 <= splits; s += 8) {
    float v[8][VEC];
#pragma unroll
    for (int u = 0; u < 8; ++u) {
      const float* p = slab + (size_t)(s + u) * mn + i;
      if constexpr (VEC == 4) {
        const float4 t = *reinterpret_cast<const float4*>(p);
        v[u][0] = t.x; v[u][1] = t.y; v[u][2] = t.z; v[u][3] = t.w;
      } else {
        v[u][0] = *p;
      }
    }
#pragma unroll
    for (int u = 0; u < 8; ++u)
#pragma unroll
      for (int k = 0; k < VEC; ++k) acc[k] += v[u][k];
  }
  for (; s < splits; ++s)
#pragma unroll
    for (int k = 0; k < VEC; ++k) acc[k] += slab[(size_t)s * mn + i + k];
  const int row = (int)(i / N), col = (int)(i - (int64_t)row * N);
  if constexpr (VEC == 4) {
    *reinterpret_cast<float4*>(C + (size_t)row * ldc + col) = make_float4(acc[0], acc[1], acc[2], acc[3]);
  } else {
    C[(size_t)row * ldc + col] = acc[0];
  }
}

bool vec_ok(const float* p, int ld, int contiguous_extent) {
  return (reinterpret_cast<uintptr_t>(p) & 15u) == 0 && (ld % 4) == 0 && (contiguous_extent % 4) == 0 &&
         contiguous_extent >= 4;
}

template <class CF, bool VEC>
void launch_v(rgcn_ctx* c, bool a_kc, bool b_kc, GemmArgs& g) {
  g.tiles_m = (g.M + CF::BM - 1) / CF::BM;
  g.tiles_n = (g.N + CF::BN - 1) / CF::BN;
  const int gx = g.swizzle == 2 ? ((g.tiles_m + 7) / 8) * 8 * g.tiles_n : g.tiles_m * g.tiles_n * g.splits;
  dim3 grid((unsigned)gx, (unsigned)g.batch.groups), block(CF::NT);
  static_assert((64 * CF::BN / 4) % CF::NT == 0 && CF::TM * 32 <= 64, "epilogue staging geometry");
  if (a_kc && !b_kc) hipLaunchKernelGGL((k_gemm_f32<true, false, VEC, CF>), grid, block, 0, c->stream, g);
  else if (a_kc && b_kc) hipLaunchKernelGGL((k_gemm_f32<true, true, VEC, CF>), grid, block, 0, c->stream, g);
  else hipLaunchKernelGGL((k_gemm_f32<false, false, VEC, CF>), grid, block, 0, c->stream, g);
}
template <class CF>
void launch(rgcn_ctx* c, bool a_kc, bool b_kc, GemmArgs& g, bool vec) {
  if (vec) launch_v<CF, true>(c, a_kc, b_kc, g); else launch_v<CF, false>(c, a_kc, b_kc, g);
}

}

rgcn_status gemm_f32(rgcn_ctx* c, const char* tag, bool a_kc, bool b_kc, int M, int N, int K,
                     const float* A, int lda, const float* B, int ldb, float* C, int ldc,
                     int split_k, const GemmBatch* batch, double prof_scale) {
  if (M <= 0 || N <= 0) return RGCN_OK;
  const int groups = batch ? batch->groups : 1;
  if (a_kc == false && b_kc == true) RGCN_FAIL(c, RGCN_ERR_UNSUPPORTED, "gemm TT form not instantiated");
  const int bk = 16;
  GemmArgs g;
  g.A = A; g.B = B; g.M = M; g.N = N; g.K = K; g.lda = lda; g.ldb = ldb;
  const bool vec = vec_ok(A, lda, a_kc ? K : M) && vec_ok(B, ldb, b_kc ? K : N) &&
                   (!batch || (batch->strideA % 4 == 0 && batch->strideB % 4 == 0));
  g.swizzle = 1;
  g.zeros = c->zeros;
  if (batch) g.batch = *batch;
  if (batch && batch->limit != nullptr && !batch->limit_on_k && split_k <= 1) g.swizzle = 2;
  if (split_k < 1) split_k = 1;
  int kps = (K + split_k - 1) / split_k;
  kps = ((kps + bk - 1) / bk) * bk;
  if (kps < bk) kps = bk;
  split_k = K > 0 ? (K + kps - 1) / kps : 1;
  g.k_per_split = kps;
  g.splits = split_k;
  const bool slabs = split_k > 1;
  if (slabs) {
    if ((size_t)groups * split_k * M * N > c->slab_floats) RGCN_FAIL(c, RGCN_ERR_STATE, "internal: split-K slab too small");
    g.C = c->slab; g.ldc = N;
    g.batch.strideC = (size_t)split_k * M * N;
  } else {
    g.C = C; g.ldc = ldc;
  }
  g.vecC = ((reinterpret_cast<uintptr_t>(g.C) & 15u) == 0 && g.ldc % 4 == 0 && N % 4 == 0) ? 1 : 0;
  {
    ProfScope ps(c, tag, prof_scale * groups * 4.0 * ((double)M * K + (double)K * N + (double)M * N),
                 prof_scale * groups * 2.0 * M * N * K);
    if (c->gemm_mode != 0) {
      RGCN_HIP(c, gemm_bf16x3_launch(c, c->gemm_mode, a_kc, b_kc, vec, M, N, K, A, lda, B, ldb, g.C, g.ldc,
                                     g.k_per_split, g.splits, g.swizzle, g.vecC, &g.batch));
    } else {
      launch<Cfg<128, 128, 16, 4, 2>>(c, a_kc, b_kc, g, vec);
    }
    RGCN_HIP(c, hipGetLastError());
  }
  if (slabs) {
    const int64_t mn = (int64_t)M * N;
    ProfScope ps(c, "splitk_reduce", 4.0 * groups * mn * (split_k + 1), 0);
    const size_t gsc = batch ? batch->strideC : 0;
    if (N % 4 == 0 && ldc % 4 == 0 && (reinterpret_cast<uintptr_t>(C) & 15u) == 0 && gsc % 4 == 0)
      hipLaunchKernelGGL((k_splitk_reduce<4>), dim3((unsigned)((mn / 4 + 255) / 256), (unsigned)groups), dim3(256), 0,
                         c->stream, c->slab, C, M, N, ldc, split_k, gsc);
    else
      hipLaunchKernelGGL((k_splitk_reduce<1>), dim3((unsigned)((mn + 255) / 256), (unsigned)groups), dim3(256), 0,
                         c->stream, c->slab, C, M, N, ldc, split_k, gsc);
    RGCN_HIP(c, hipGetLastError());
  }
  return RGCN_OK;
}

}
```

### relationprediction_amd/csrc/gemm_split.h

```cpp
#ifndef RGCN_GEMM_SPLIT_H_
#define RGCN_GEMM_SPLIT_H_

#include <type_traits>
#include <utility>

#include "rgcn_internal.h"

namespace rgcn {
namespace gx {

using f32x16 = __attribute__((ext_vector_type(16))) float;
using bf16x8 = __attribute__((ext_vector_type(8))) __bf16;
using u32x4 = __attribute__((ext_vector_type(4))) uint32_t;
using f32x4 = __attribute__((ext_vector_type(4))) float;

struct XArgs {
  const float* A;
  const float* B;
  float* C;
  const float* zeros;
  int M, N, K;
  int lda, ldb, ldc;
  int k_per_split;
  int tiles_m, tiles_n, splits;
  int swizzle;
  int vecC;
  GemmBatch batch;
  const u32x4* bfrag;
  int nt32;
};

inline hipError_t set_dynamic_lds(const void* kern, int bytes, int device, uint64_t& done) {
  const uint64_t bit = device < 64 ? 1ull << device : 0;
  if (done & bit) return hipSuccess;
  const hipError_t e = hipFuncSetAttribute(kern, hipFuncAttributeMaxDynamicSharedMemorySize, bytes);
  if (e == hipSuccess) done |= bit;
  return e;
}

constexpr int BM = 128, BN = 128, BK = 16, NTH = 256;
constexpr int KC_LD = 12;
constexpr int RC_LD = 136;
constexpr int KC_PLANE = 128 * KC_LD;
constexpr int RC_PLANE = 8 * RC_LD;
constexpr int EPI_LD = BN + 4;

using bf16x2 = __attribute__((ext_vector_type(2))) __bf16;
using f32x2 = __attribute__((ext_vector_type(2))) float;

template <int I0, int I1>
__device__ __forceinline__ uint32_t split_level(f32x4& v0, f32x4& v1, uint32_t negmask = 0u) {
  const float x0 = v0[I0], x1 = v1[I1];
  const f32x2 f = {__builtin_bit_cast(float, __builtin_bit_cast(uint32_t, x0) ^ negmask),
                   __builtin_bit_cast(float, __builtin_bit_cast(uint32_t, x1) ^ negmask)};
  const uint32_t u = __builtin_bit_cast(uint32_t, __builtin_convertvector(f, bf16x2));
  v0[I0] = f[0] - __builtin_bit_cast(float, u << 16);
  v1[I1] = f[1] - __builtin_bit_cast(float, u & 0xffff0000u);
  return u;
}
__device__ __forceinline__ uint32_t split_last(float x0, float x1) {
  const f32x2 f = {x0, x1};
  return __builtin_bit_cast(uint32_t, __builtin_convertvector(f, bf16x2));
}

__device__ __forceinline__ void lds_barrier() {
  asm volatile("s_waitcnt lgkmcnt(0)\n\ts_barrier" ::: "memory");
}

template <int I, int N, class F>
__device__ __forceinline__ void static_for(F& f) {
  if constexpr (I < N) {
    f(std::integral_constant<int, I>{});
    static_for<I + 1, N>(f);
  }
}
__host__ __device__ constexpr int bfrag_nt32(int N) { return 8 * ((N + 255) / 256); }

}
}
#endif
```

### relationprediction_amd/csrc/rgcn_devtools.hip

```cpp
#include "rgcn_api_internal.h"

using namespace rgcn;

extern "C" {

#ifdef RGCN_DEVTOOLS
namespace {
__global__ void k_xcd_of_block(int32_t* out) {
  uint32_t id;
  asm volatile("s_getreg_b32 %0, hwreg(HW_REG_XCC_ID)" : "=s"(id));
  if (threadIdx.x == 0) out[blockIdx.x] = (int32_t)(id & 0xf);
}
}

rgcn_status rgcn_debug_xcd_map(rgcn_ctx* c, int32_t n_blocks, int32_t* out_host) {
  RGCN_NEED(c);
  if (n_blocks <= 0 || !out_host) RGCN_FAIL(c, RGCN_ERR_INVALID, "bad arguments");
  int32_t* dev = nullptr;
  RGCN_TRY(dmalloc(c, &dev, (size_t)n_blocks));
  hipLaunchKernelGGL(k_xcd_of_block, dim3((unsigned)n_blocks), dim3(256), 0, c->stream, dev);
  rgcn_status s = hipGetLastError() == hipSuccess ? RGCN_OK : RGCN_ERR_HIP;
  if (s == RGCN_OK) s = to_host(c, out_host, dev, sizeof(int32_t) * (size_t)n_blocks);
  (void)hipFree(dev);
  return s;
}

rgcn_status rgcn_debug_gemm(rgcn_ctx* c, int32_t ta, int32_t tb, int32_t M, int32_t N, int32_t K,
                            int32_t split_k, const float* a_host, const float* b_host, float* c_host) {
  RGCN_NEED(c);
  if (M <= 0 || N <= 0 || K <= 0 || !a_host || !b_host || !c_host) RGCN_FAIL(c, RGCN_ERR_INVALID, "bad arguments");
  if (ta && tb) RGCN_FAIL(c, RGCN_ERR_UNSUPPORTED, "TT form not instantiated");
  float *A = nullptr, *B = nullptr, *C = nullptr;
  rgcn_status s = RGCN_OK;
  do {
    if ((s = dmalloc(c, &A, (size_t)M * K, false)) != RGCN_OK) break;
    if ((s = dmalloc(c, &B, (size_t)K * N, false)) != RGCN_OK) break;
    if ((s = dmalloc(c, &C, (size_t)M * N)) != RGCN_OK) break;
    if ((s = to_dev(c, A, a_host, sizeof(float) * (size_t)M * K)) != RGCN_OK) break;
    if ((s = to_dev(c, B, b_host, sizeof(float) * (size_t)K * N)) != RGCN_OK) break;
    int sk = split_k > 0 ? split_k : auto_split_k(M, N, K);
    if ((size_t)sk * M * N > c->slab_floats) sk = 1;
    s = gemm_f32(c, "debug_gemm", ta == 0, tb != 0, M, N, K, A, ta ? M : K, B, tb ? K : N, C, N, sk);
    if (s != RGCN_OK) break;
    s = to_host(c, c_host, C, sizeof(float) * (size_t)M * N);
  } while (0);
  if (A) (void)hipFree(A);
  if (B) (void)hipFree(B);
  if (C) (void)hipFree(C);
  return s;
}

rgcn_status rgcn_debug_gemm_presplit(rgcn_ctx* c, int32_t tb, int32_t M, int32_t N, int32_t K, int32_t iters,
                                     const float* a_host, const float* b_host, float* c_host, float* avg_ms) {
  RGCN_NEED(c);
  if (M <= 0 || N <= 0 || K <= 0 || !a_host || !b_host || !c_host) RGCN_FAIL(c, RGCN_ERR_INVALID, "bad arguments");
  float *A = nullptr, *B = nullptr, *C = nullptr;
  void* F = nullptr;
  rgcn_status s = RGCN_OK;
  do {
    if ((s = dmalloc(c, &A, (size_t)M * K, false)) != RGCN_OK) break;
    if ((s = dmalloc(c, &B, (size_t)K * N, false)) != RGCN_OK) break;
    if ((s = dmalloc(c, &C, (size_t)M * N)) != RGCN_OK) break;
    if (hipMalloc(&F, 16 * gemm_bfrag_words(K, N)) != hipSuccess) { s = RGCN_ERR_NOMEM; break; }
    if ((s = to_dev(c, A, a_host, sizeof(float) * (size_t)M * K)) != RGCN_OK) break;
    if ((s = to_dev(c, B, b_host, sizeof(float) * (size_t)K * N)) != RGCN_OK) break;
    const PresplitJob pj{B, F, tb ? K : N, K, N, tb ? 1 : 0};
    if ((s = gemm_presplit_b(c, &pj, 1)) != RGCN_OK) break;
    GemmBatch gb;
    gb.bfrag = F;
    gb.wide = 1;
    s = gemm_f32(c, "debug_gemm", true, tb != 0, M, N, K, A, K, B, tb ? K : N, C, N, 1, &gb);
    if (s != RGCN_OK) break;
    if ((s = to_host(c, c_host, C, sizeof(float) * (size_t)M * N)) != RGCN_OK) break;
    if (iters > 0 && avg_ms) {
      if ((s = rgcn_timer_start(c)) != RGCN_OK) break;
      for (int it = 0; it < iters && s == RGCN_OK; ++it)
        s = gemm_f32(c, "debug_gemm", true, tb != 0, M, N, K, A, K, B, tb ? K : N, C, N, 1, &gb);
      if (s != RGCN_OK) break;
      float ms = 0.f;
      if ((s = rgcn_timer_stop(c, &ms)) != RGCN_OK) break;
      *avg_ms = ms / iters;
    }
  } while (0);
  if (A) (void)hipFree(A);
  if (B) (void)hipFree(B);
  if (C) (void)hipFree(C);
  if (F) (void)hipFree(F);
  return s;
}

rgcn_status rgcn_debug_gemm_time(rgcn_ctx* c, int32_t ta, int32_t tb, int32_t M, int32_t N, int32_t K,
                                 int32_t split_k, int32_t iters, const float* a_host,
                                 const float* b_host, float* avg_ms) {
  RGCN_NEED(c);
  if (M <= 0 || N <= 0 || K <= 0 || iters <= 0 || !a_host || !b_host || !avg_ms)
    RGCN_FAIL(c, RGCN_ERR_INVALID, "bad arguments");
  if (ta && tb) RGCN_FAIL(c, RGCN_ERR_UNSUPPORTED, "TT form not instantiated");
  float *A = nullptr, *B = nullptr, *C = nullptr;
  rgcn_status s = RGCN_OK;
  do {
    if ((s = dmalloc(c, &A, (size_t)M * K, false)) != RGCN_OK) break;
    if ((s = dmalloc(c, &B, (size_t)K * N, false)) != RGCN_OK) break;
    if ((s = dmalloc(c, &C, (size_t)M * N)) != RGCN_OK) break;
    if ((s = to_dev(c, A, a_host, sizeof(float) * (size_t)M * K)) != RGCN_OK) break;
    if ((s = to_dev(c, B, b_host, sizeof(float) * (size_t)K * N)) != RGCN_OK) break;
    int sk = split_k > 0 ? split_k : auto_split_k(M, N, K);
    if ((size_t)sk * M * N > c->slab_floats) sk = 1;
    for (int it = 0; it < 3 && s == RGCN_OK; ++it)
      s = gemm_f32(c, "debug_gemm", ta == 0, tb != 0, M, N, K, A, ta ? M : K, B, tb ? K : N, C, N, sk);
    if (s != RGCN_OK) break;
    if ((s = rgcn_timer_start(c)) != RGCN_OK) break;
    for (int it = 0; it < iters && s == RGCN_OK; ++it)
      s = gemm_f32(c, "debug_gemm", ta == 0, tb != 0, M, N, K, A, ta ? M : K, B, tb ? K : N, C, N, sk);
    if (s != RGCN_OK) break;
    float ms = 0.f;
    if ((s = rgcn_timer_stop(c, &ms)) != RGCN_OK) break;
    *avg_ms = ms / iters;
  } while (0);
  if (A) (void)hipFree(A);
  if (B) (void)hipFree(B);
  if (C) (void)hipFree(C);
  return s;
}

#endif

}
```

### relationprediction_amd/csrc/rgcn_internal.h

```cpp
#pragma once

#include <hip/hip_runtime.h>

#include <cstdint>
#include <cstdio>
#include <cstdlib>
#include <cstring>
#include <string>
#include <vector>

#include "../../include/rgcn.h"

namespace rgcn {

#ifdef RGCN_DEVTOOLS
inline int knob(const char* name, int dflt) {
  const char* s = getenv(name);
  return s ? atoi(s) : dflt;
}
#else
constexpr int knob(const char*, int dflt) { return dflt; }
#endif

void set_global_error(const std::string& s);

#define RGCN_HIP(ctx, expr)                                                                      \
  do {                                                                                           \
    hipError_t _e = (expr);                                                                      \
    if (_e != hipSuccess) {                                                                      \
      (ctx)->err = std::string(#expr) + ": " + hipGetErrorString(_e) + " (" __FILE__ ":" +       \
                   std::to_string(__LINE__) + ")";                                               \
      return RGCN_ERR_HIP;                                                                       \
    }                                                                                            \
  } while (0)

#define RGCN_TRY(expr)                       \
  do {                                       \
    rgcn_status _s = (expr);                 \
    if (_s != RGCN_OK) return _s;            \
  } while (0)

#define RGCN_FAIL(ctx, code, msg)            \
  do {                                       \
    (ctx)->err = (msg);                      \
    return (code);                           \
  } while (0)

__host__ __device__ inline uint64_t splitmix64_mix(uint64_t z) {
  z = (z ^ (z >> 30)) * 0xBF58476D1CE4E5B9ull;
  z = (z ^ (z >> 27)) * 0x94D049BB133111EBull;
  return z ^ (z >> 31);
}
__host__ __device__ inline uint32_t drop_bits(uint64_t seed, uint32_t layer, uint64_t idx) {
  return (uint32_t)(splitmix64_mix(seed + 0x9E3779B97F4A7C15ull * (idx + ((uint64_t)layer << 44) + 1ull)) >> 40);
}
struct DropKey {
  uint32_t k0, k1;
};
__host__ __device__ inline DropKey drop_key_of(uint64_t seed, uint32_t layer) {
  const uint64_t z = splitmix64_mix(seed + 0x9E3779B97F4A7C15ull * (((uint64_t)layer << 44) + 1ull));
  return DropKey{(uint32_t)z, (uint32_t)(z >> 32)};
}
__host__ __device__ inline uint32_t drop_bits24(const DropKey& k, uint64_t idx) {
  const uint32_t hi = (uint32_t)(idx >> 32);
  uint32_t x = (uint32_t)idx ^ k.k0 ^ ((hi << 16) | (hi >> 16));
  x ^= x >> 16;
  x *= 0x7feb352du;
  x += k.k1;
  x ^= x >> 15;
  x *= 0x846ca68bu;
  x ^= x >> 16;
  return x >> 8;
}

enum DropMode { DROP_NONE = 0, DROP_RNG = 1, DROP_MASK = 2 };

constexpr int kLongRow = 32;
constexpr int kGiantRow = 2048;
constexpr int kAuxStreams = 3;

struct DropSpec {
  int32_t mode;
  uint32_t layer;
  uint32_t thresh;
  float inv_keep;
  uint64_t seed;
  const uint8_t* mask;
  const uint64_t* seed_offset;
};

#if defined(__HIPCC__)
__device__ __forceinline__ DropKey drop_key(const DropSpec& ds) {
  if (ds.mode != DROP_RNG) return DropKey{0u, 0u};
  return drop_key_of(ds.seed + (ds.seed_offset ? *ds.seed_offset : 0ull), ds.layer);
}
__device__ __forceinline__ float drop_factor(const DropSpec& ds, const DropKey& key, size_t idx) {
  if (ds.mode == DROP_NONE) return 1.0f;
  if (ds.mode == DROP_RNG) return drop_bits24(key, idx) < ds.thresh ? ds.inv_keep : 0.0f;
  return ds.mask[idx] ? ds.inv_keep : 0.0f;
}
__device__ __forceinline__ float drop_factor(const DropSpec& ds, size_t idx) { return drop_factor(ds, drop_key(ds), idx); }
#endif

struct ProfRec {
  const char* name;
  hipEvent_t e0, e1;
  double bytes, flops, cbytes;
};
struct ProfAgg {
  std::string name;
  int64_t calls;
  double ms, bytes, flops, cbytes;
};

enum ParamLayout {
  LAYOUT_PLAIN = 0,
  LAYOUT_BLOCK_T = 1,
  LAYOUT_BASIS_T = 2
};

struct Param {
  std::string name;
  int32_t ndim;
  int64_t shape[4];
  int64_t count;
  float* val;
  float* grad;
  int32_t layout;
  bool no_grad = false;
};

struct LayerBufs {
  float* wrel = nullptr;
  float* grel = nullptr;
  float* coef = nullptr;
  float* gcoef = nullptr;
  float* wself = nullptr;
  float* gwself = nullptr;
  float* bias = nullptr;
  float* gbias = nullptr;
  void *wself_nn = nullptr, *wself_nt = nullptr, *wrel_nn = nullptr, *wrel_nt = nullptr;
  float* wtile = nullptr;
  uint64_t wtile_version = ~0ull;
};

struct GraphBufs {
  int32_t* triples = nullptr;
  const int32_t* cur = nullptr;
  int64_t E = 0;
  int32_t* indeg = nullptr;
  int32_t* outdeg = nullptr;
  int32_t* counters = nullptr;
  size_t counters_bytes = 0;
  int32_t* row_ptr = nullptr;
  int32_t* long_rows = nullptr;
  int32_t *giant_rows = nullptr, *giant_first = nullptr, *giant_cnt = nullptr, *piece_row = nullptr, *piece_k = nullptr;
  int32_t* ngiant = nullptr;
  int32_t giant_cap = 0, piece_cap = 0;
  bool giant_on = false;
  uint32_t *row_key = nullptr, *row_key_s = nullptr;
  int32_t* row_order = nullptr;
  uint16_t* row_tab = nullptr;
  int32_t* nlong = nullptr;
  int32_t long_cap = 0;
  int32_t* rel_ptr = nullptr;
  int chunk = 48;
  int32_t* chunk_ptr = nullptr;
  int32_t* cum_in = nullptr;
  int32_t* cum_out = nullptr;
  uint32_t *keyv = nullptr, *keyv_s = nullptr, *keyr = nullptr, *keyr_s = nullptr;
  int32_t *valv = nullptr, *permv = nullptr, *valr = nullptr, *permr = nullptr;
  int32_t* pos = nullptr;
  int32_t *m_src = nullptr, *m_dst = nullptr, *m_dslot = nullptr, *m_sslot = nullptr;
  int32_t *d_src = nullptr, *d_rel = nullptr, *s_dst = nullptr, *s_rel = nullptr;
  float *d_norm = nullptr, *s_norm = nullptr;
  float* m_norm = nullptr;
  int32_t *has_dir = nullptr, *unit_ptr = nullptr, *unit_rows = nullptr;
  int64_t units_host = -1;
  uint32_t *keyv_t = nullptr, *keyr_t = nullptr;
  uint16_t *tablev = nullptr, *tabler = nullptr;
  uint32_t *keyd = nullptr, *keyd_s = nullptr, *keyd_t = nullptr;
  int32_t *vald = nullptr, *permd = nullptr;
  uint16_t* tabled = nullptr;
  const int32_t* pf_tri = nullptr;
  int64_t pf_E = -1;
  int64_t pf_keep = -1;
  uint64_t pf_eseed = 0;
  bool pf_valid = false;
  hipEvent_t ev_ready = nullptr;
  hipEvent_t ev_free = nullptr;
  bool ready_in_capture = false, free_in_capture = false;
  int32_t* owner = nullptr;
  int32_t* errflag = nullptr;
  bool ready = false;
};

struct DecoderBufs {
  int64_t maxN = 0;
  int32_t N = 0;
  int64_t N_total = 0;
  const int32_t* tiled_X = nullptr;
  int64_t tiled_period = 0, tiled_N = 0;
  int32_t* perm_pos = nullptr;
  const int32_t* X = nullptr;
  uint32_t *keyv = nullptr, *keyv_s = nullptr, *keyr = nullptr, *keyr_s = nullptr;
  int32_t *valv = nullptr, *permv = nullptr, *valr = nullptr, *permr = nullptr;
  int32_t *row_ptr = nullptr, *rel_ptr = nullptr, *chunk_ptr = nullptr;
  int32_t *e_other = nullptr, *e_rel = nullptr, *e_trip = nullptr;
  int32_t *long_rows = nullptr, *nlong = nullptr;
  int32_t *long_first = nullptr, *long_cnt = nullptr;
  int32_t *piece_row = nullptr, *piece_k = nullptr;
  float* piece_slab = nullptr;
  int32_t long_cap = 0, piece_cap = 0, max_chunks = 0, energy_blocks = 0;
  float *dx = nullptr, *loss_part = nullptr, *slab = nullptr;
  float *cb = nullptr, *rb = nullptr, *e_g = nullptr;
  uint32_t *row_key = nullptr, *row_key_s = nullptr;
  int32_t* row_order = nullptr;
  uint16_t* row_tab = nullptr;
  int32_t nbands = 0, cus = 0;
  double* loss = nullptr;
  uint32_t *keyv_t = nullptr, *keyr_t = nullptr;
  uint16_t *tablev = nullptr, *tabler = nullptr;
  uint32_t *keyd = nullptr, *keyd_s = nullptr, *keyd_t = nullptr;
  int32_t *vald = nullptr, *permd = nullptr;
  uint16_t* tabled = nullptr;
  hipEvent_t ev_ready = nullptr;
  bool loss_valid = false;
};

struct NeighborhoodBufs {
  int64_t n = 0;
  int32_t* triples = nullptr;
  int32_t *adj_other = nullptr, *adj_end = nullptr;
  int32_t *seg_v = nullptr, *seg_beg = nullptr, *seg_end = nullptr;
  int32_t nseg = 0;
  int32_t launches = 64;
  int32_t* comp = nullptr;
  uint8_t* comp_state = nullptr;
  uint32_t* dist = nullptr;
  unsigned long long* tkey = nullptr;
  uint32_t* hist = nullptr;
  unsigned long long* state = nullptr;
  int32_t* changed = nullptr;
  uint32_t* bcnt = nullptr;
  void* params = nullptr;
  hipGraph_t draw_graph = nullptr;
  hipGraphExec_t draw_exec = nullptr;
  hipStream_t capture_stream = nullptr;
  hipEvent_t ev_draw = nullptr;
  hipStream_t last_draw_stream = nullptr;
  std::vector<int32_t> comp_h;
  std::vector<int64_t> comp_edges_h;
  std::vector<uint8_t> comp_state_h;
  int32_t ncomp = 0;
};

struct OptimizerState {
  bool configured = false;
  float lr = 0.01f, beta1 = 0.9f, beta2 = 0.999f, eps = 1e-8f, max_norm = 0.f;
  int64_t t = 0;
  std::vector<float*> m, v;
  float* part = nullptr;
  size_t part_cap = 0;
  float* state = nullptr;
  float* shard_sq = nullptr;
  bool norm_pending = false;
};

}

struct rgcn_ctx {
  rgcn_config cfg;
  int V = 0, R = 0, d = 0, L = 0, nb = 0, sd = 0, kind = 0, B = 0;
  int rank = 0, world = 1;
  bool onehot = false;
  int row_lo = 0, row_hi = 0;
  int shard_rows = 0;
  int V_pad = 0;
  float* repl_grads = nullptr;
  size_t repl_grads_floats = 0;
  hipEvent_t ev_gather = nullptr;
  bool gather_pending = false;
  hipStream_t stream = nullptr;
  hipStream_t main_stream = nullptr;
  hipStream_t aux[rgcn::kAuxStreams] = {nullptr, nullptr, nullptr};
  hipEvent_t ev_fork = nullptr, ev_join[rgcn::kAuxStreams] = {nullptr, nullptr, nullptr};
  bool use_aux = true;
  bool aux_dirty[rgcn::kAuxStreams] = {false, false, false};
  int fuse = 1;
  uint64_t weights_version = 1;
  bool dw_pending = false;
  enum { SIDE_NONE = 0, SIDE_RECORDED = 1, SIDE_READS_JOINED = 2 };
  int side_state = SIDE_NONE;
  bool defer_end_joins = false;
  std::string err;

  std::vector<rgcn::Param> params;
  std::vector<rgcn::LayerBufs> layers;
  float *w_emb = nullptr, *g_emb = nullptr, *b_emb = nullptr, *gb_emb = nullptr;
  float *w_rel = nullptr, *g_rel = nullptr;
  rgcn::DecoderBufs dec;
  rgcn::NeighborhoodBufs nbr;
  rgcn::OptimizerState opt;

  std::vector<float*> H;
  float* self_buf = nullptr;
  float* exch = nullptr;
  float* dbuf[2] = {nullptr, nullptr};
  float* dsbuf[2] = {nullptr, nullptr};
  float* msgbuf = nullptr;
  float* msgbuf2 = nullptr;
  std::vector<float*> zsave;
  float* aggbuf = nullptr;
  float* slab = nullptr;
  size_t slab_floats = 0;
  float* slab_dw = nullptr;
  size_t slab_dw_floats = 0;
  float* stage = nullptr;
  size_t stage_floats = 0;
  uint8_t* masks = nullptr;
  float* colsum_part = nullptr;
  size_t colsum_part_floats = 0;
  int colsum_half = 0;
  int32_t colsum_parts = 0;
  float* zeros = nullptr;

  rgcn::GraphBufs g;
  rgcn::GraphBufs g_alt;
  hipStream_t pf_stream = nullptr;
  int aux_priority = 0, pf_priority = 0;
  static constexpr int kStageSlots = 8;
  static constexpr size_t kStageBytes = (size_t)1 << 20;
  uint8_t* stage_host = nullptr;
  uint8_t* readback_host = nullptr;
  hipEvent_t stage_done[kStageSlots] = {};
  int stage_next = 0;
  int chunk = 48;
  int gemm_mode = 0;
  int msg_block = 0, msg_slots = 0;

  uint64_t frag_version = ~0ull;
  bool frag_fresh = false;
  bool wtile_fresh = false;
  bool fwd_done = false;
  int fwd_train = 0;
  uint64_t seed = 0;
  bool explicit_masks = false;
  const float* bwd_D = nullptr;
  const float* bwd_dS = nullptr;
  int bwd_layer = 0;
  bool capturing = false;
  bool use_aux_before_capture = true;
  bool cap_pf_forked = false;
  uint64_t* replay_counter = nullptr;
  hipEvent_t ev_step_begin = nullptr;
  bool step_begin_in_capture = false;
  std::vector<hipGraphExec_t> graphs;
  std::vector<hipGraph_t> graph_defs;
  float* giant_slab = nullptr;
  float *rank_q = nullptr, *rank_s = nullptr;
  int32_t* rank_bad = nullptr;
  float* rank_thr = nullptr;
  int64_t rank_max = 0;
  float* dcodes_own = nullptr;

  void* comm = nullptr;
  bool prof_on = false;
  bool dropout_lds_configured = false;
  std::vector<rgcn::ProfRec> prof;
  std::vector<hipEvent_t> event_pool;
  std::vector<rgcn::ProfAgg> prof_agg;
  hipEvent_t t0 = nullptr, t1 = nullptr;
};

namespace rgcn {

inline unsigned order_event_flags(const rgcn_ctx* c, bool kernel_only = false) {
  return hipEventDisableTiming | (kernel_only && c->world == 1 ? hipEventDisableSystemFence : 0u);
}

struct StreamScope {
  rgcn_ctx* c;
  hipStream_t saved;
  bool active;
  StreamScope(rgcn_ctx* ctx, int k, bool in_capture = false);
  ~StreamScope();
};
rgcn_status stream_join(rgcn_ctx* c, int k);
inline float* colsum_scratch(const rgcn_ctx* c) { return c->colsum_part + (size_t)c->colsum_half * c->colsum_part_floats; }

struct ProfScope {
  rgcn_ctx* c;
  int idx;
  ProfScope(rgcn_ctx* ctx, const char* name, double bytes, double flops, double compulsory = -1.0);
  ~ProfScope();
};

rgcn_status graph_alloc(rgcn_ctx* c, const GraphBufs* share);
void graph_free(rgcn_ctx* c);
rgcn_status graph_build(rgcn_ctx* c, const int32_t* triples_dev, int64_t E);
rgcn_status graph_build_dropout(rgcn_ctx* c, const int32_t* batch_dev, int64_t n, int64_t keep, uint64_t seed,
                                const uint8_t* keep_mask_dev);

struct SortSpec {
  const uint32_t* key_in;
  uint32_t* key_out;
  int32_t* val_out;
  uint32_t* key_tmp;
  int32_t* val_tmp;
  int32_t* pos_out;
  uint16_t* table;
  int64_t n;
  uint32_t max_key;
};
size_t sort_table_elems(size_t n);
rgcn_status sort_pairs(rgcn_ctx* c, const char* tag, int njobs, const SortSpec* specs);

struct GemmBatch {
  int groups = 1;
  size_t strideA = 0, strideB = 0, strideC = 0;
  const int32_t* limit = nullptr;
  int limit_stride = 1;
  int limit_on_k = 0;
  const void* bfrag = nullptr;
  size_t strideBfrag = 0;
  int wide = 0;
};
size_t gemm_bfrag_words(int K, int N);
struct PresplitJob {
  const float* B;
  void* F;
  int ldb, K, N, b_kc;
};
rgcn_status gemm_presplit_b(rgcn_ctx* c, const PresplitJob* jobs, int n);

rgcn_status gemm_f32(rgcn_ctx* c, const char* tag, bool a_kc, bool b_kc, int M, int N, int K,
                     const float* A, int lda, const float* B, int ldb, float* C, int ldc,
                     int split_k, const GemmBatch* batch = nullptr, double prof_scale = 1.0);

hipError_t gemm_bf16x3_launch(rgcn_ctx* c, int terms, bool a_kc, bool b_kc, bool vec, int M, int N, int K,
                              const float* A, int lda, const float* B, int ldb, float* C, int ldc,
                              int k_per_split, int splits, int swizzle, int vecC, const GemmBatch* batch = nullptr);
hipError_t gemm_bf16x3_w8_launch(rgcn_ctx* c, int terms, int M, int N, int K, const float* A, int lda, float* C, int ldc,
                                 int swizzle, int vecC, const GemmBatch& batch);

rgcn_status block_geometry(rgcn_ctx* c);
rgcn_status block_msg_forward(rgcn_ctx* c, int layer, const float* Hin, float* Ybuf);
rgcn_status block_msg_backward(rgcn_ctx* c, int layer, const float* Hin, const float* D, float* Zbuf);
rgcn_status block_dw_reduce(rgcn_ctx* c, int layer);
rgcn_status block_to_device_layout(rgcn_ctx* c, const float* host_layout_dev, float* dst, int R);
rgcn_status block_from_device_layout(rgcn_ctx* c, const float* src, float* host_layout_dev, int R);

struct CombineArgs;
bool block_rows_available(const rgcn_ctx* c);
size_t block_rows_weight_floats(const rgcn_ctx* c);
rgcn_status block_rows(rgcn_ctx* c, const char* tag, int layer, bool backward, const float* X, const CombineArgs& ca);

rgcn_status basis_aggregate_forward(rgcn_ctx* c, int layer, const float* Hin, float* Z);
struct CombineArgs;
rgcn_status basis_backward_gather(rgcn_ctx* c, int layer, const float* dZ, const CombineArgs& ca,
                                  bool with_messages);
rgcn_status basis_dcoef(rgcn_ctx* c, int layer, const float* Hin, const float* dZ);
rgcn_status basis_dcoef_reduce(rgcn_ctx* c, int layer);
double basis_units(rgcn_ctx* c);
rgcn_status basis_gather_units(rgcn_ctx* c, const float* D, float* Dc);
rgcn_status basis_to_device_layout(rgcn_ctx* c, const float* host_layout_dev, float* dst);
rgcn_status basis_from_device_layout(rgcn_ctx* c, const float* src, float* host_layout_dev);

rgcn_status onehot_forward(rgcn_ctx* c, float* out);
rgcn_status onehot_backward_tables(rgcn_ctx* c, const float* D);
rgcn_status onehot_dcoef(rgcn_ctx* c, const float* D);

struct CombineArgs {
  float* out;
  float* out2;
  const float* base;
  const float* add;
  const float* add_units = nullptr;
  const int32_t* unit_ptr = nullptr;
  const float* msg;
  const int32_t* row_ptr;
  const int32_t* long_rows;
  const int32_t* nlong;
  const int32_t* giant_rows = nullptr;
  const int32_t* giant_first = nullptr;
  const int32_t* giant_cnt = nullptr;
  const int32_t* piece_row = nullptr;
  const int32_t* piece_k = nullptr;
  const int32_t* ngiant = nullptr;
  float* giant_slab = nullptr;
  const float* gate;
  int32_t V, d;
  int32_t relu;
  int32_t row_lo, row_hi;
  int32_t v_begin = 0, v_count = -1;
  int32_t colsum = 0;
  DropSpec drop;
  DropSpec drop2;
};
rgcn_status combine(rgcn_ctx* c, const char* tag, const CombineArgs& a, double alg_bytes);
rgcn_status combine_giant_finish(rgcn_ctx* c, const CombineArgs& a);
rgcn_status column_sum_giant_rows(rgcn_ctx* c, const float* out, float* part);
rgcn_status column_sum_finish(rgcn_ctx* c, float* out, int nparts, int cols);
rgcn_status input_forward(rgcn_ctx* c);
rgcn_status scale_dropout(rgcn_ctx* c, const float* in, float* out, const DropSpec& ds);
rgcn_status column_sum(rgcn_ctx* c, const float* in, float* out, int rows, int cols);
rgcn_status relu_copy(rgcn_ctx* c, const float* in, float* out, int64_t n, int relu);
rgcn_status materialize_mask(rgcn_ctx* c, const DropSpec& ds, uint8_t* out_dev, int64_t n);

DropSpec make_drop(const rgcn_ctx* c, int layer, bool active);

rgcn_status negative_sample(rgcn_ctx* c, const int32_t* batch_dev, int64_t n, int rate, uint64_t seed, int32_t* X,
                            float* Y);
rgcn_status decoder_reserve(rgcn_ctx* c, int64_t max_triples);
void decoder_free(rgcn_ctx* c);
rgcn_status decoder_prepare(rgcn_ctx* c, const int32_t* X_dev, int64_t N, int64_t N_total = 0);
rgcn_status decoder_compute(rgcn_ctx* c, const float* codes, const float* Y_dev, float reg_param,
                            float* dcodes_drop = nullptr, const DropSpec* drop = nullptr);
rgcn_status decoder_allreduce(rgcn_ctx* c);
rgcn_status optimizer_step(rgcn_ctx* c);
rgcn_status optimizer_norm_partial(rgcn_ctx* c);
rgcn_status optimizer_apply(rgcn_ctx* c);
rgcn_status neighborhood_reserve(rgcn_ctx* c, const int32_t* triples_host, int64_t n);
rgcn_status neighborhood_sample(rgcn_ctx* c, int64_t sample_size, uint64_t seed, int32_t* batch_out_dev,
                                bool on_prefetch_stream);
void neighborhood_free(rgcn_ctx* c);
rgcn_status rank_reserve(rgcn_ctx* c, int64_t max_queries);
void rank_free(rgcn_ctx* c);
rgcn_status rank_compute(rgcn_ctx* c, const int32_t* X_dev, int64_t N, int predict_object, const int64_t* filt_ptr,
                         const int32_t* filt_idx, int32_t* raw_out, int32_t* filt_out);
rgcn_status topk_compute(rgcn_ctx* c, const int32_t* X_dev, int64_t N, int predict_object, int k,
                         const int64_t* excl_ptr, const int32_t* excl_idx, int32_t* idx_out, float* energy_out);
void optimizer_free(rgcn_ctx* c);

rgcn_status comm_unique_id(uint8_t id[128]);
rgcn_status comm_init(rgcn_ctx* c, const uint8_t id[128]);
rgcn_status comm_allreduce(rgcn_ctx* c, float* buf, int64_t count);
rgcn_status comm_reduce_scatter(rgcn_ctx* c, float* buf, int64_t count_per_rank);
rgcn_status comm_all_gather(rgcn_ctx* c, float* buf, int64_t count_per_rank);
rgcn_status comm_info(rgcn_ctx* c, int32_t* ranks, int32_t* rank, int32_t* device);
void comm_destroy(rgcn_ctx* c);

}
```

### relationprediction_amd/csrc/rgcn_schedule.hip

```cpp
#include "rgcn_api_internal.h"

namespace rgcn {

rgcn_status fwd_begin(rgcn_ctx* c, int train, uint64_t seed, const uint8_t* masks_host) {
  if (!c->g.ready) RGCN_FAIL(c, RGCN_ERR_STATE, "rgcn_forward before rgcn_set_graph");
  RGCN_TRY(join_side_reads(c));
  c->fwd_done = false;
  c->frag_fresh = false;
  c->wtile_fresh = false;
  c->fwd_train = train ? 1 : 0;
  c->seed = seed;
  c->explicit_masks = false;
  if (train && masks_host) {
    const size_t n = (size_t)c->L * c->V * c->d;
    if (!c->masks) RGCN_TRY(dmalloc(c, &c->masks, n, false));
    RGCN_TRY(to_dev(c, c->masks, masks_host, n));
    c->explicit_masks = true;
  }
  if (c->onehot) return RGCN_OK;
  return input_forward(c);
}

static rgcn_status wait_gather(rgcn_ctx* c) {
  if (c->gather_pending) {
    RGCN_HIP(c, hipStreamWaitEvent(c->stream, c->ev_gather, 0));
    if (c->stream == c->main_stream) c->gather_pending = false;
  }
  return RGCN_OK;
}
static rgcn_status gather_rows(rgcn_ctx* c, float* buf) {
  StreamScope side(c, 1);
  RGCN_TRY(comm_all_gather(c, buf, (int64_t)c->shard_rows * c->d));
  if (side.active) {
    RGCN_HIP(c, hipEventRecord(c->ev_gather, c->aux[1]));
    c->gather_pending = true;
  }
  return RGCN_OK;
}

static bool rows_layer(const rgcn_ctx* c) { return c->fuse == 1 && block_rows_available(c); }

static rgcn_status refresh_weight_fragments(rgcn_ctx* c) {
  if (c->gemm_mode == 0) return RGCN_OK;
  if (c->capturing ? c->frag_fresh : c->frag_version == c->weights_version) return RGCN_OK;
  std::vector<PresplitJob> jobs;
  const int d = c->d, Bd = c->B * c->d;
  for (int l = 1; l <= c->L; ++l) {
    LayerBufs& lb = c->layers[l];
    if (!lb.wself_nn || !lb.wself_nt) continue;
    jobs.push_back(PresplitJob{lb.wself, lb.wself_nn, d, d, d, 0});
    jobs.push_back(PresplitJob{lb.wself, lb.wself_nt, d, d, d, 1});
    if (c->kind == RGCN_KIND_BASIS && lb.wrel_nn && lb.wrel_nt)
      for (int g = 0; g < 2; ++g) {
        const float* W = lb.wrel + (size_t)g * Bd * d;
        jobs.push_back(PresplitJob{W, static_cast<char*>(lb.wrel_nn) + 16 * g * gemm_bfrag_words(Bd, d), d, Bd, d, 0});
        jobs.push_back(PresplitJob{W, static_cast<char*>(lb.wrel_nt) + 16 * g * gemm_bfrag_words(d, Bd), d, d, Bd, 1});
      }
  }
  if (!jobs.empty()) RGCN_TRY(gemm_presplit_b(c, jobs.data(), (int)jobs.size()));
  c->frag_fresh = true;
  c->frag_version = c->capturing ? ~0ull : c->weights_version;
  return RGCN_OK;
}
static rgcn_status self_loop_batch(rgcn_ctx* c, int l, bool transposed, GemmBatch* b) {
  *b = GemmBatch();
  RGCN_TRY(refresh_weight_fragments(c));
  if (c->gemm_mode != 0) b->bfrag = transposed ? c->layers[l].wself_nt : c->layers[l].wself_nn;
  b->wide = transposed ? 0 : 1;
  return RGCN_OK;
}

static GemmBatch basis_batch(const rgcn_ctx* c, size_t strideA, size_t strideB, size_t strideC, bool limit_on_k) {
  GemmBatch b;
  b.groups = 2;
  b.strideA = strideA; b.strideB = strideB; b.strideC = strideC;
  b.limit = c->g.unit_ptr + c->V;
  b.limit_stride = c->V + 1;
  b.limit_on_k = limit_on_k ? 1 : 0;
  return b;
}
static double basis_unit_share(rgcn_ctx* c) { return basis_units(c) / (2.0 * c->V); }

rgcn_status fwd_layer_partial(rgcn_ctx* c, int l) {
  if (l < 1 || l > c->L) RGCN_FAIL(c, RGCN_ERR_INVALID, "layer out of range");
  if (c->onehot && l == 1) return onehot_forward(c, c->H[1]);
  const float* Hin = c->H[l - 1];
  const int d = c->d, V = c->V;
  const int lo = c->world > 1 ? c->row_lo : 0, hi = c->world > 1 ? c->row_hi : V;
  float* dst = c->world > 1 ? c->exch : c->H[l];
  const double Mmsg = 2.0 * c->g.E / c->world;
  GemmBatch sb;
  RGCN_TRY(self_loop_batch(c, l, false, &sb));
  if (c->kind == RGCN_KIND_BLOCK && rows_layer(c)) {
    RGCN_TRY(gemm_f32(c, "gemm_self_fwd", true, false, hi - lo, d, d, Hin + (size_t)lo * d, d, c->layers[l].wself, d,
                      c->self_buf + (size_t)lo * d, d, 1, &sb));
    RGCN_TRY(wait_gather(c));
    CombineArgs a;
    a.add = nullptr; a.msg = nullptr; a.row_ptr = nullptr; a.long_rows = nullptr; a.nlong = nullptr;
    a.out = dst; a.out2 = nullptr; a.base = c->self_buf; a.gate = nullptr; a.V = V; a.d = d;
    a.relu = (c->world == 1 && l < c->L) ? 1 : 0;
    a.row_lo = lo; a.row_hi = hi;
    a.drop = make_drop(c, l, true);
    a.drop2 = make_drop(c, l, false);
    RGCN_TRY(block_rows(c, "block_rows_fwd", l, false, Hin, a));
  } else if (c->kind == RGCN_KIND_BLOCK) {
    {
      StreamScope side(c, 0);
      RGCN_TRY(gemm_f32(c, "gemm_self_fwd", true, false, hi - lo, d, d, Hin + (size_t)lo * d, d,
                        c->layers[l].wself, d, c->self_buf + (size_t)lo * d, d, 1, &sb));
    }
    RGCN_TRY(wait_gather(c));
    RGCN_TRY(block_msg_forward(c, l, Hin, c->msgbuf));
    RGCN_TRY(stream_join(c, 0));
    CombineArgs a;
    a.add = nullptr;
    a.out = dst; a.out2 = nullptr; a.base = c->self_buf; a.msg = c->g.E > 0 ? c->msgbuf : nullptr;
    a.row_ptr = c->g.row_ptr; a.long_rows = c->g.long_rows; a.nlong = c->g.nlong; a.gate = nullptr; a.V = V; a.d = d;
    a.relu = (c->world == 1 && l < c->L) ? 1 : 0;
    a.row_lo = lo; a.row_hi = hi;
    a.drop = make_drop(c, l, true);
    a.drop2 = make_drop(c, l, false);
    RGCN_TRY(combine(c, "combine_fwd", a, 4.0 * d * (2.0 * V + Mmsg) + 4.0 * V));
  } else {
    const int Bd = c->B * d;
    {
      StreamScope side(c, 1);
      RGCN_TRY(gemm_f32(c, "gemm_self_fwd", true, false, hi - lo, d, d, Hin + (size_t)lo * d, d,
                        c->layers[l].wself, d, c->self_buf + (size_t)lo * d, d, 1, &sb));
    }
    RGCN_TRY(wait_gather(c));
    RGCN_TRY(basis_aggregate_forward(c, l, Hin, c->zsave[l]));
    GemmBatch gb = basis_batch(c, (size_t)V * Bd, (size_t)Bd * d, (size_t)V * d, false);
    RGCN_TRY(refresh_weight_fragments(c));
    if (c->gemm_mode != 0) gb.bfrag = c->layers[l].wrel_nn;
    gb.strideBfrag = gemm_bfrag_words(Bd, d);
    gb.wide = 1;
    RGCN_TRY(gemm_f32(c, "gemm_basis_fwd", true, false, V, d, Bd, c->zsave[l], Bd, c->layers[l].wrel, d,
                      c->aggbuf, d, 1, &gb, basis_unit_share(c)));
    RGCN_TRY(stream_join(c, 1));
    CombineArgs a;
    a.add = nullptr;
    a.add_units = c->aggbuf; a.unit_ptr = c->g.unit_ptr;
    a.out = dst; a.out2 = nullptr; a.base = c->self_buf; a.msg = nullptr; a.row_ptr = nullptr;
    a.long_rows = nullptr; a.nlong = nullptr; a.gate = nullptr; a.V = V; a.d = d;
    a.relu = (c->world == 1 && l < c->L) ? 1 : 0;
    a.row_lo = lo; a.row_hi = hi;
    a.drop = make_drop(c, l, true);
    a.drop2 = make_drop(c, l, false);
    RGCN_TRY(combine(c, "combine_fwd", a, 4.0 * d * (2.0 * V + 2.0 * V * basis_unit_share(c)) + 8.0 * V));
  }
  return RGCN_OK;
}

rgcn_status fwd_layer_finish(rgcn_ctx* c, int l) {
  if (l < 1 || l > c->L) RGCN_FAIL(c, RGCN_ERR_INVALID, "layer out of range");
  if (c->world > 1)
    RGCN_TRY(relu_copy(c, c->exch, c->H[l], (int64_t)c->V * c->d, l < c->L ? 1 : 0));
  if (l == c->L) c->fwd_done = true;
  return RGCN_OK;
}

static bool deferred_schedule(const rgcn_ctx* c) {
  return c->defer_end_joins && c->kind == RGCN_KIND_BLOCK && c->fuse == 1 && block_rows_available(c) && c->world == 1 &&
         c->g.E <= 65536 && c->use_aux && !c->capturing && c->L >= 2 && c->stream == c->main_stream;
}

rgcn_status bwd_begin(rgcn_ctx* c, const float* dcodes_dev, const float* ds_ready) {
  if (!c->fwd_done) RGCN_FAIL(c, RGCN_ERR_STATE, "rgcn_backward needs a completed rgcn_forward on the current graph");
  if (!dcodes_dev) RGCN_FAIL(c, RGCN_ERR_INVALID, "dcodes is NULL");
  if (!(c->side_state == rgcn_ctx::SIDE_READS_JOINED && deferred_schedule(c))) RGCN_TRY(join_abandoned_side_work(c));
  c->bwd_layer = c->L;
  c->bwd_D = dcodes_dev;
  DropSpec ds = make_drop(c, c->L, true);
  if (ds.mode != DROP_NONE && ds_ready != nullptr) {
    c->bwd_dS = ds_ready;
  } else if (ds.mode != DROP_NONE) {
    RGCN_TRY(scale_dropout(c, dcodes_dev, c->dsbuf[c->L & 1], ds));
    c->bwd_dS = c->dsbuf[c->L & 1];
  } else {
    c->bwd_dS = dcodes_dev;
  }
  return RGCN_OK;
}

rgcn_status bwd_layer_partial(rgcn_ctx* c, int l) {
  if (l != c->bwd_layer || l < 1) RGCN_FAIL(c, RGCN_ERR_STATE, "backward layers must run L..1 in order");
  if (c->onehot && l == 1) {
    {
      StreamScope side(c, 0);
      RGCN_TRY(onehot_dcoef(c, c->bwd_D));
    }
    RGCN_TRY(relu_copy(c, c->bwd_dS, c->layers[1].gwself, (int64_t)c->V * c->d, 0));
    RGCN_TRY(onehot_backward_tables(c, c->bwd_D));
    return stream_join(c, 0);
  }
  const float* Hin = c->H[l - 1];
  const int d = c->d, V = c->V;
  const int lo = c->world > 1 ? c->row_lo : 0, hi = c->world > 1 ? c->row_hi : V;
  const int rows = hi - lo;
  LayerBufs& lb = c->layers[l];
  const double Mmsg = 2.0 * c->g.E / c->world;
  const bool narrow_dw = c->kind == RGCN_KIND_BASIS || rows >= 32768;

  CombineArgs a;
  a.add = nullptr;
  a.base = c->self_buf; a.msg = nullptr; a.row_ptr = nullptr; a.long_rows = nullptr; a.nlong = nullptr;
  a.V = V; a.d = d; a.relu = 0; a.row_lo = lo; a.row_hi = hi;
  a.drop = make_drop(c, l, false);
  if (c->world == 1) {
    a.out = (l - 1 == 0) ? c->g_emb : c->dbuf[(l - 1) & 1];
    a.colsum = (l - 1 == 0) ? 1 : 0;
    a.drop2 = make_drop(c, l - 1, l - 1 >= 1);
    a.out2 = a.drop2.mode != DROP_NONE ? c->dsbuf[(l - 1) & 1] : nullptr;
    a.gate = Hin;
  } else {
    a.out = c->exch; a.out2 = nullptr; a.gate = nullptr; a.drop2 = make_drop(c, l, false);
  }

  if (c->dw_pending) {
    RGCN_TRY(stream_join(c, 0));
    c->dw_pending = false;
  }
  auto self_dw = [&]() {
    return gemm_f32(c, "gemm_self_dw", false, false, d, d, rows, Hin + (size_t)lo * d, d, c->bwd_dS + (size_t)lo * d, d,
                    lb.gwself, d, auto_split_k(d, d, rows, narrow_dw));
  };
  GemmBatch sbt;
  RGCN_TRY(self_loop_batch(c, l, true, &sbt));
  auto self_dh = [&]() {
    return gemm_f32(c, "gemm_self_dh", true, true, rows, d, d, c->bwd_dS + (size_t)lo * d, d, lb.wself, d,
                    c->self_buf + (size_t)lo * d, d, 1, &sbt);
  };
  bool defer_joins = false;
  if (c->kind == RGCN_KIND_BLOCK && rows_layer(c)) {
    const bool minibatch = c->world == 1 && c->g.E <= 65536;
    if (minibatch && c->use_aux) {
      {
        StreamScope side(c, 1);
        RGCN_TRY(self_dw());
      }
      RGCN_TRY(self_dh());
      {
        StreamScope side(c, 0);
        RGCN_TRY(block_msg_backward(c, l, Hin, c->bwd_D, nullptr));
        RGCN_TRY(block_dw_reduce(c, l));
      }
      RGCN_TRY(block_rows(c, "block_rows_bwd", l, true, c->bwd_D, a));
      defer_joins = l == 2;
      if (l == 1 && deferred_schedule(c)) {
        RGCN_TRY(record_side_done(c));
        defer_joins = true;
      }
      if (!defer_joins) RGCN_TRY(stream_join_both(c));
    } else if (minibatch) {
      RGCN_TRY(block_msg_backward(c, l, Hin, c->bwd_D, nullptr));
      {
        StreamScope side(c, 1, true);
        RGCN_TRY(block_dw_reduce(c, l));
        RGCN_TRY(self_dw());
      }
      RGCN_TRY(self_dh());
      RGCN_TRY(block_rows(c, "block_rows_bwd", l, true, c->bwd_D, a));
    } else {
      {
        StreamScope side(c, 0);
        RGCN_TRY(wait_gather(c));
        RGCN_TRY(block_msg_backward(c, l, Hin, c->bwd_D, nullptr));
        RGCN_TRY(block_dw_reduce(c, l));
        c->dw_pending = side.active;
      }
      {
        StreamScope side(c, 1);
        RGCN_TRY(self_dw());
      }
      RGCN_TRY(self_dh());
      RGCN_TRY(wait_gather(c));
      RGCN_TRY(block_rows(c, "block_rows_bwd", l, true, c->bwd_D, a));
    }
  } else if (c->kind == RGCN_KIND_BLOCK) {
    {
      StreamScope side(c, 0);
      RGCN_TRY(wait_gather(c));
      RGCN_TRY(block_msg_backward(c, l, Hin, c->bwd_D, c->msgbuf));
      if (side.active) RGCN_HIP(c, hipEventRecord(c->ev_join[0], c->aux[0]));
      RGCN_TRY(block_dw_reduce(c, l));
    }
    RGCN_TRY(self_dh());
    {
      StreamScope side(c, 1);
      RGCN_TRY(self_dw());
    }
    if (c->use_aux) RGCN_HIP(c, hipStreamWaitEvent(c->main_stream, c->ev_join[0], 0));
    a.msg = c->g.E > 0 ? c->msgbuf : nullptr;
    a.row_ptr = c->g.row_ptr;
    a.long_rows = c->g.long_rows;
    a.nlong = c->g.nlong;
    RGCN_TRY(combine(c, "combine_bwd", a, 4.0 * d * ((a.out2 ? 4.0 : 3.0) * V + Mmsg) + 4.0 * V));
  } else {
    const int Bd = c->B * d;
    RGCN_TRY(wait_gather(c));
    RGCN_TRY(basis_gather_units(c, c->bwd_D, c->aggbuf));
    {
      StreamScope side(c, 1);
      RGCN_TRY(self_dw());
      const GemmBatch gk = basis_batch(c, (size_t)V * Bd, (size_t)V * d, (size_t)Bd * d, true);
      RGCN_TRY(gemm_f32(c, "gemm_basis_dw", false, false, Bd, d, V, c->zsave[l], Bd, c->aggbuf, d, lb.grel, d,
                        auto_split_k(2 * Bd, d, V), &gk, basis_unit_share(c)));
    }
    RGCN_TRY(self_dh());
    GemmBatch gm = basis_batch(c, (size_t)V * d, (size_t)Bd * d, (size_t)V * Bd, false);
    RGCN_TRY(refresh_weight_fragments(c));
    if (c->gemm_mode != 0) gm.bfrag = lb.wrel_nt;
    gm.strideBfrag = gemm_bfrag_words(d, Bd);
    RGCN_TRY(gemm_f32(c, "gemm_basis_dz", true, true, V, Bd, d, c->aggbuf, d, lb.wrel, d, c->msgbuf2, Bd, 1, &gm,
                      basis_unit_share(c)));
    RGCN_TRY(basis_dcoef(c, l, Hin, c->msgbuf2));
    RGCN_TRY(basis_backward_gather(c, l, c->msgbuf2, a, true));
  }
  if (!defer_joins) RGCN_TRY(stream_join(c, 1));
  return RGCN_OK;
}

rgcn_status bwd_layer_finish(rgcn_ctx* c, int l) {
  if (l != c->bwd_layer || l < 1) RGCN_FAIL(c, RGCN_ERR_STATE, "backward layers must run L..1 in order");
  float* out = (l - 1 == 0) ? c->g_emb : c->dbuf[(l - 1) & 1];
  DropSpec d2 = make_drop(c, l - 1, l - 1 >= 1);
  float* out2 = d2.mode != DROP_NONE ? c->dsbuf[(l - 1) & 1] : nullptr;
  if (c->world > 1) {
    CombineArgs a;
    a.add = nullptr;
    a.out = out; a.out2 = out2; a.base = c->exch; a.msg = nullptr; a.row_ptr = nullptr; a.long_rows = nullptr; a.nlong = nullptr;
    a.gate = c->H[l - 1]; a.V = c->V; a.d = c->d; a.relu = 0; a.row_lo = 0; a.row_hi = c->V;
    a.drop = make_drop(c, l, false);
    a.drop2 = d2;
    RGCN_TRY(combine(c, "combine_bwd_finish", a, 4.0 * c->d * (out2 ? 4.0 : 3.0) * c->V));
  }
  c->bwd_D = out;
  c->bwd_dS = out2 ? out2 : out;
  c->bwd_layer = l - 1;
  return RGCN_OK;
}

rgcn_status bwd_end(rgcn_ctx* c) {
  if (c->bwd_layer != 0) RGCN_FAIL(c, RGCN_ERR_STATE, "rgcn_backward_end before all layers ran");
  if (c->onehot) {
    if (c->side_state != rgcn_ctx::SIDE_NONE) RGCN_TRY(join_abandoned_side_work(c));
    c->dw_pending = false;
    return stream_join(c, 0);
  }
  if (c->defer_end_joins && c->side_state == rgcn_ctx::SIDE_RECORDED && c->stream == c->main_stream && c->colsum_parts > 0) {
    {
      StreamScope side(c, 1);
      if (!side.active) RGCN_FAIL(c, RGCN_ERR_HIP, "internal: fork onto side stream 1 failed");
      RGCN_TRY(column_sum_finish(c, c->gb_emb, c->colsum_parts, c->d));
    }
    RGCN_HIP(c, hipStreamWaitEvent(c->aux[1], c->ev_join[0], 0));
    c->colsum_half ^= 1;
    c->colsum_parts = 0;
    c->dw_pending = false;
    return RGCN_OK;
  }
  if (c->side_state != rgcn_ctx::SIDE_NONE) RGCN_TRY(join_abandoned_side_work(c));
  if (c->colsum_parts > 0) RGCN_TRY(column_sum_finish(c, c->gb_emb, c->colsum_parts, c->d));
  else RGCN_TRY(column_sum(c, c->g_emb, c->gb_emb, c->V, c->d));
  c->colsum_parts = 0;
  c->dw_pending = false;
  return stream_join(c, 0);
}

static rgcn_status fwd_exchange(rgcn_ctx* c, int l) {
  const int64_t chunk = (int64_t)c->shard_rows * c->d;
  RGCN_TRY(comm_reduce_scatter(c, c->exch, chunk));
  const size_t off = (size_t)c->rank * chunk;
  RGCN_TRY(relu_copy(c, c->exch + off, c->H[l] + off, chunk, l < c->L ? 1 : 0));
  RGCN_TRY(gather_rows(c, c->H[l]));
  if (l == c->L) {
    RGCN_TRY(wait_gather(c));
    c->fwd_done = true;
  }
  return RGCN_OK;
}

static rgcn_status bwd_exchange(rgcn_ctx* c, int l) {
  const int64_t chunk = (int64_t)c->shard_rows * c->d;
  RGCN_TRY(comm_reduce_scatter(c, c->exch, chunk));
  float* out = (l - 1 == 0) ? c->g_emb : c->dbuf[(l - 1) & 1];
  DropSpec d2 = make_drop(c, l - 1, l - 1 >= 1);
  float* out2 = d2.mode != DROP_NONE ? c->dsbuf[(l - 1) & 1] : nullptr;
  CombineArgs a;
  a.add = nullptr;
  a.out = out; a.out2 = out2; a.base = c->exch; a.msg = nullptr; a.row_ptr = nullptr; a.long_rows = nullptr; a.nlong = nullptr;
  a.gate = c->H[l - 1]; a.V = c->V; a.d = c->d; a.relu = 0; a.row_lo = c->row_lo; a.row_hi = c->row_hi;
  a.v_begin = c->row_lo; a.v_count = c->row_hi - c->row_lo;
  a.drop = make_drop(c, l, false);
  a.drop2 = d2;
  if (a.v_count > 0) RGCN_TRY(combine(c, "combine_bwd_finish", a, 4.0 * c->d * (out2 ? 4.0 : 3.0) * a.v_count));
  RGCN_TRY(gather_rows(c, out));
  c->bwd_D = out;
  c->bwd_dS = out2 ? out2 : out;
  c->bwd_layer = l - 1;
  return RGCN_OK;
}

rgcn_status forward_all(rgcn_ctx* c, int train, uint64_t seed, const uint8_t* masks) {
  if (c->world > 1 && !c->comm)
    RGCN_FAIL(c, RGCN_ERR_STATE, "world > 1: call rgcn_comm_init first (or drive the phase API yourself)");
  RGCN_TRY(fwd_begin(c, train, seed, masks));
  for (int l = 1; l <= c->L; ++l) {
    RGCN_TRY(fwd_layer_partial(c, l));
    if (c->world > 1) RGCN_TRY(fwd_exchange(c, l));
    else RGCN_TRY(fwd_layer_finish(c, l));
  }
  return RGCN_OK;
}

rgcn_status backward_all(rgcn_ctx* c, const float* dcodes_dev, const float* ds_ready) {
  if (c->world > 1 && !c->comm)
    RGCN_FAIL(c, RGCN_ERR_STATE, "world > 1: call rgcn_comm_init first (or drive the phase API yourself)");
  RGCN_TRY(bwd_begin(c, dcodes_dev, ds_ready));
  for (int l = c->L; l >= 1; --l) {
    RGCN_TRY(bwd_layer_partial(c, l));
    if (c->world > 1) RGCN_TRY(bwd_exchange(c, l));
    else RGCN_TRY(bwd_layer_finish(c, l));
  }
  if (c->world > 1) {
    RGCN_TRY(wait_gather(c));
    RGCN_TRY(comm_allreduce(c, c->repl_grads, (int64_t)c->repl_grads_floats));
  }
  return bwd_end(c);
}

}
```

Before: 30.90 million edges/s.

## Fuse input embedding bias+ReLU into layer-1 self-loop GEMM A-operand prologue

```diff
diff --git a/include/rgcn_devtools.h b/include/rgcn_devtools.h
--- a/include/rgcn_devtools.h
+++ b/include/rgcn_devtools.h
@@ -21,6 +21,10 @@
 rgcn_status rgcn_debug_gemm_presplit(rgcn_ctx* ctx, int32_t trans_b, int32_t M, int32_t N, int32_t K, int32_t iters,
                                      const float* a_host, const float* b_host, float* c_host, float* avg_ms);
 
+rgcn_status rgcn_debug_gemm_prologue(rgcn_ctx* ctx, int32_t wide, int32_t prologue, int32_t M, int32_t N, int32_t K,
+                                     int32_t lda, int32_t row_limit, const float* a_host, const float* bias_host,
+                                     const float* b_host, float* a_out_host, float* c_host);
+
 rgcn_status rgcn_debug_xcd_map(rgcn_ctx* ctx, int32_t n_blocks, int32_t* out_host);
 
 #if defined(__GNUC__)
diff --git a/relationprediction_amd/_native.py b/relationprediction_amd/_native.py
--- a/relationprediction_amd/_native.py
+++ b/relationprediction_amd/_native.py
@@ -137,6 +137,8 @@
                                              C.POINTER(C.c_float)]),
     "rgcn_debug_gemm_time": (C.c_int32, [_P, C.c_int32, C.c_int32, C.c_int32, C.c_int32, C.c_int32, C.c_int32,
                                          C.c_int32, _P, _P, C.POINTER(C.c_float)]),
+    "rgcn_debug_gemm_prologue": (C.c_int32, [_P, C.c_int32, C.c_int32, C.c_int32, C.c_int32, C.c_int32, C.c_int32,
+                                             C.c_int32, _P, _P, _P, _P, _P]),
 }
 _lib_devtools = None
 
@@ -712,6 +714,19 @@
                                                       _ptr(out), C.byref(ms)))
         return (out, float(ms.value)) if iters else out
 
+    def debug_gemm_prologue(self, a, bias, b, a_out, wide=True, prologue=True, row_limit=-1):
+        a = np.ascontiguousarray(a, dtype=np.float32)
+        b = np.ascontiguousarray(b, dtype=np.float32)
+        bias = np.ascontiguousarray(bias, dtype=np.float32)
+        out_a = np.array(a_out, dtype=np.float32, order="C", copy=True)
+        M, lda = a.shape
+        K, N = b.shape
+        assert bias.shape == (K,) and out_a.shape == (M, lda)
+        out = np.empty((M, N), dtype=np.float32)
+        self._check(self.lib.rgcn_debug_gemm_prologue(self.ctx, int(bool(wide)), int(bool(prologue)), M, N, K, lda,
+                                                      int(row_limit), _ptr(a), _ptr(bias), _ptr(b), _ptr(out_a), _ptr(out)))
+        return out, out_a
+
     def debug_xcd_map(self, n_blocks):
         out = np.zeros(int(n_blocks), dtype=np.int32)
         self._check(self.lib.rgcn_debug_xcd_map(self.ctx, int(n_blocks), _ptr(out)))
diff --git a/relationprediction_amd/build.py b/relationprediction_amd/build.py
--- a/relationprediction_amd/build.py
+++ b/relationprediction_amd/build.py
@@ -19,7 +19,7 @@
            "elementwise.hip", "decoder.hip", "optimizer.hip", "ranking.hip", "sampler.hip", "neighborhood.hip", "comm.hip"]
 HEADERS = [os.path.join(CSRC, "rgcn_internal.h"), os.path.join(CSRC, "rgcn_api_internal.h"), os.path.join(CSRC, "gemm_split.h"), os.path.join(ROOT, "include", "rgcn.h"),
            os.path.join(ROOT, "include", "rgcn_devtools.h")]
-DEVTOOLS_SOURCES = ["rgcn_api.hip", "rgcn_devtools.hip", "comm.hip", "decoder.hip", "gemm_bf16x3.hip", "gemm_bf16x3_w8.hip"]
+DEVTOOLS_SOURCES = ["rgcn_api.hip", "rgcn_schedule.hip", "rgcn_devtools.hip", "comm.hip", "decoder.hip", "gemm_bf16x3.hip", "gemm_bf16x3_w8.hip"]
 NO_PACKED_FP32 = ["-Xclang", "-target-feature", "-Xclang", "-packed-fp32-ops"]
 FLAGS = ["--offload-arch=" + ARCH, "-O3", "-std=c++17", "-fPIC", "-fvisibility=hidden", "-Wall",
          "-Wno-unused-function"] + NO_PACKED_FP32
diff --git a/relationprediction_amd/csrc/gemm_bf16x3.hip b/relationprediction_amd/csrc/gemm_bf16x3.hip
--- a/relationprediction_amd/csrc/gemm_bf16x3.hip
+++ b/relationprediction_amd/csrc/gemm_bf16x3.hip
@@ -109,8 +109,11 @@
   return __builtin_bit_cast(bf16x8, v);
 }
 
-template <bool A_KC, bool B_KC, bool VEC, int TERMS, bool B_PRE = false>
+constexpr int PRO_OFF = 2 * 3 * KC_PLANE;
+constexpr int PRO_BYTES = (PRO_MAX_KT + 1) * BK * 4;
+template <bool A_KC, bool B_KC, bool VEC, int TERMS, bool B_PRE = false, bool APRO = false>
 __global__ void __launch_bounds__(NTH, 2) k_gemm_bf16x3(XArgs g) {
+  static_assert(!APRO || (B_PRE && A_KC && VEC), "the prologue exists for the pre-split-weight NN form");
   constexpr int PA = A_KC ? KC_PLANE : RC_PLANE, PB = B_KC ? KC_PLANE : RC_PLANE;
   constexpr int TA = 3 * PA, TB = B_PRE ? 0 : 3 * PB;
   extern __shared__ __attribute__((aligned(16))) uint32_t lds[];
@@ -215,6 +218,27 @@
       }
     }
   };
+  float* const lbias = reinterpret_cast<float*>(lds) + PRO_OFF;
+  const bool writes_a = APRO && n0 == 0 && g.batch.a_out != nullptr;
+  auto apro = [&](int tile, f32x4 (&xa)[2]) {
+    if constexpr (APRO) {
+#pragma unroll
+      for (int p = 0; p < 2; ++p) {
+        const int f = threadIdx.x + NTH * p;
+        const int row = m0 + (f >> 2), kq = (f & 3) * 4;
+        const f32x4 b = *reinterpret_cast<const f32x4*>(lbias + min(tile, nkt) * BK + kq);
+#pragma unroll
+        for (int e = 0; e < 4; ++e) xa[p][e] = fmaxf(xa[p][e] + b[e], 0.f);
+        const int k = tile * BK + kq;
+        if (writes_a && row < Mlim && k < ke)
+          *reinterpret_cast<f32x4*>(g.batch.a_out + (size_t)grp * g.batch.strideA + (size_t)row * g.lda + k) = xa[p];
+      }
+    }
+  };
+  if constexpr (APRO) {
+    for (int i = threadIdx.x; i < (nkt + 1) * BK; i += NTH) lbias[i] = i < ke ? g.batch.a_bias[i] : -__builtin_inff();
+    __syncthreads();
+  }
   auto sstore = [&](uint32_t* buf, f32x4 (&xa)[2], f32x4 (&xb)[2]) {
     SplitRegs st;
     split_chunks<A_KC, PA, 0, 12>(xa, st, buf);
@@ -254,6 +278,7 @@
     const uint32_t negmask = (sign_group(kt + 1) & 1) ? 0x80000000u : 0u;
     if constexpr (WALK) gwalk(ra[P], rb[P]); else gload(ks + (kt + 2) * BK, ra[P], rb[P]);
     if constexpr (B_PRE) bfetch(kt + 1, fbp[1 - P]);
+    apro(kt + 1, ra[1 - P]);
     const uint32_t* a_lds = lds + P * (TA + TB);
     const uint32_t* b_lds = a_lds + TA;
     uint32_t* nxt = lds + (1 - P) * (TA + TB);
@@ -295,6 +320,7 @@
   if (nkt > 0) {
     gload(ks, ra[0], rb[0]);
     if constexpr (B_PRE) bfetch(0, fbp[0]);
+    apro(0, ra[0]);
     sstore(lds, ra[0], rb[0]);
     gload(ks + BK, ra[1], rb[1]);
   }
@@ -368,10 +394,11 @@
   return tiles > epi ? tiles : epi;
 }
 
-template <bool A_KC, bool B_KC, bool VEC, int TERMS, bool B_PRE = false>
+template <bool A_KC, bool B_KC, bool VEC, int TERMS, bool B_PRE = false, bool APRO = false>
 hipError_t launch_one(rgcn_ctx* c, const XArgs& g) {
-  constexpr size_t bytes = lds_bytes(A_KC, B_KC, B_PRE);
-  auto kern = k_gemm_bf16x3<A_KC, B_KC, VEC, TERMS, B_PRE>;
+  static_assert(!APRO || lds_bytes(A_KC, B_KC, B_PRE) == PRO_OFF * 4, "the bias copy starts where the tile buffers end");
+  constexpr size_t bytes = lds_bytes(A_KC, B_KC, B_PRE) + (APRO ? PRO_BYTES : 0);
+  auto kern = k_gemm_bf16x3<A_KC, B_KC, VEC, TERMS, B_PRE, APRO>;
   static uint64_t configured = 0;
   const hipError_t e = set_dynamic_lds(reinterpret_cast<const void*>(kern), (int)bytes, c->cfg.device, configured);
   if (e != hipSuccess) return e;
@@ -383,6 +410,9 @@
 template <bool VEC, int TERMS>
 hipError_t launch_form(rgcn_ctx* c, bool a_kc, bool b_kc, const XArgs& g) {
   if constexpr (VEC) {
+    if constexpr (TERMS != 3) {
+      if (g.bfrag != nullptr && a_kc && g.batch.a_bias != nullptr) return launch_one<true, true, true, TERMS, true, true>(c, g);
+    }
     if (g.bfrag != nullptr && a_kc) return launch_one<true, true, true, TERMS, true>(c, g);
   }
   if (a_kc && !b_kc) return launch_one<true, false, VEC, TERMS>(c, g);
@@ -427,6 +457,14 @@
 
 }
 
+bool gemm_a_prologue_ok(const rgcn_ctx* c, int N, int K, const float* A, int lda, const float* B, int ldb, const void* bfrag) {
+  auto vec = [](const float* p, int ld, int extent) {
+    return (reinterpret_cast<uintptr_t>(p) & 15u) == 0 && ld % 4 == 0 && extent % 4 == 0 && extent >= 4;
+  };
+  (void)B; (void)ldb; (void)N;
+  return (c->gemm_mode == 6 || c->gemm_mode == 9) && bfrag != nullptr && vec(A, lda, K) && (K + BK - 1) / BK <= PRO_MAX_KT;
+}
+
 size_t gemm_bfrag_words(int K, int N) {
   return (size_t)((K + BK - 1) / BK) * bfrag_nt32(N) * 192;
 }
@@ -463,6 +501,9 @@
   g.tiles_m = (M + BM - 1) / BM;
   g.tiles_n = (N + BN - 1) / BN;
   g.nt32 = bfrag_nt32(N);
+  if (g.batch.a_bias != nullptr &&
+      !(g.bfrag != nullptr && !b_kc && g.batch.limit_on_k == 0 && (terms == 6 || terms == 9) && (K + BK - 1) / BK <= PRO_MAX_KT))
+    return hipErrorInvalidValue;
   const int w8 = knob("RGCN_GEMM_W8", 1);
   bool wide = g.batch.wide != 0;
   if (wide && g.batch.limit == nullptr) {
diff --git a/relationprediction_amd/csrc/gemm_bf16x3_w8.hip b/relationprediction_amd/csrc/gemm_bf16x3_w8.hip
--- a/relationprediction_amd/csrc/gemm_bf16x3_w8.hip
+++ b/relationprediction_amd/csrc/gemm_bf16x3_w8.hip
@@ -14,12 +14,16 @@
 constexpr int ST_SZ = A_SZ + B_SZ;
 constexpr int W_LDS_BYTES = 4 * ST_SZ;
 constexpr int WEPI_LD = WBN + 4;
+constexpr int PRO_LDS_BYTES = (PRO_MAX_KT + 1) * BK * 4;
 
 __device__ __forceinline__ void aload(f32x4& dst, const float* p) {
   asm volatile("global_load_dwordx4 %0, %1, off" : "=v"(dst) : "v"(p) : "memory");
 }
 __device__ __forceinline__ void aload_s(f32x4& dst, uint32_t voff, const float* sbase) {
   asm volatile("global_load_dwordx4 %0, %1, %2" : "=v"(dst) : "v"(voff), "s"(sbase) : "memory");
+}
+__device__ __forceinline__ void astore_s(uint32_t voff, const f32x4& v, float* sbase) {
+  asm volatile("global_store_dwordx4 %0, %1, %2" : : "v"(voff), "v"(v), "s"(sbase) : "memory");
 }
 template <int PIECE>
 __device__ __forceinline__ void dma1(uint32_t voff, const u32x4* sbase, uint32_t lds_addr) {
@@ -35,7 +39,7 @@
       : "memory");
 }
 
-template <int TERMS>
+template <int TERMS, bool APRO = false>
 __global__ void __launch_bounds__(WNTH, 2) __attribute__((amdgpu_num_vgpr(192))) k_gemm_w8(XArgs g) {
   extern __shared__ __attribute__((aligned(16))) uint32_t lds[];
 
@@ -82,6 +86,17 @@
   const float* sa = gA + (size_t)m0 * g.lda;
   const uint32_t a_off = ((uint32_t)min(arow, Mlim - 1 - m0) * (uint32_t)g.lda + 4u * aq) * 4u;
   const bool atail_ok = 4 * aq < (g.K & (BK - 1));
+  float* const lbias = reinterpret_cast<float*>(lds) + W_LDS_BYTES / 4;
+  float* so = nullptr;
+  bool st_ok = false;
+  if constexpr (APRO) {
+    for (int i = threadIdx.x; i < (nkt + 1) * BK; i += WNTH) lbias[i] = i < g.K ? g.batch.a_bias[i] : -__builtin_inff();
+    if (n0 == 0 && g.batch.a_out != nullptr) {
+      so = g.batch.a_out + (size_t)grp * g.batch.strideA + (size_t)m0 * g.lda;
+      st_ok = arow < Mlim - m0;
+    }
+    __syncthreads();
+  }
   f32x4 ra[4];
   const uint32_t a_wr = (aq >> 1) * A_HS + arow * 16 + (aq & 1) * 8;
   const u32x4* sb = g.bfrag + (size_t)grp * g.batch.strideBfrag + ((size_t)(n0 >> 5) + wave) * 192;
@@ -175,6 +190,14 @@
       if constexpr (m < 8 && m % 2 == 1) issue_part(t + 4, slot, std::integral_constant<int, m / 2>{});
       if constexpr (m < 12) read_frag(mi, st_rd, fn);
       if constexpr (m == M_WAIT) asm volatile("s_waitcnt vmcnt(8)" : "+v"(rs) : : "memory");
+      if constexpr (APRO && m == M_WAIT) {
+        const int s = t + 2;
+        const f32x4 b = *reinterpret_cast<const f32x4*>(lbias + min(s, nkt) * BK + 4 * aq);
+#pragma unroll
+        for (int e = 0; e < 4; ++e) rs[e] = fmaxf(rs[e] + b[e], 0.f);
+        if (st_ok && (s < nfull || (s < nkt && atail_ok))) astore_s(a_off, rs, so);
+        so += BK;
+      }
       if constexpr (m > M_WAIT && (m - M_WAIT) % 2 == 1 && (m - M_WAIT) / 2 < 5)
         split_piece(std::integral_constant<int, (m - M_WAIT) / 2>{}, rs, st_wr, negmask);
       __builtin_amdgcn_sched_barrier(0);
@@ -240,14 +263,15 @@
   }
 }
 
-template <int TERMS>
+template <int TERMS, bool APRO = false>
 hipError_t launch_w8(rgcn_ctx* c, const XArgs& g) {
-  auto kern = k_gemm_w8<TERMS>;
+  auto kern = k_gemm_w8<TERMS, APRO>;
+  constexpr int bytes = W_LDS_BYTES + (APRO ? PRO_LDS_BYTES : 0);
   static uint64_t configured = 0;
-  const hipError_t e = set_dynamic_lds(reinterpret_cast<const void*>(kern), W_LDS_BYTES, c->cfg.device, configured);
+  const hipError_t e = set_dynamic_lds(reinterpret_cast<const void*>(kern), bytes, c->cfg.device, configured);
   if (e != hipSuccess) return e;
   const int gx = g.swizzle == 2 ? ((g.tiles_m + 7) / 8) * 8 * g.tiles_n : g.tiles_m * g.tiles_n;
-  hipLaunchKernelGGL(kern, dim3((unsigned)gx, (unsigned)g.batch.groups), dim3(WNTH), W_LDS_BYTES, c->stream, g);
+  hipLaunchKernelGGL(kern, dim3((unsigned)gx, (unsigned)g.batch.groups), dim3(WNTH), bytes, c->stream, g);
   return hipGetLastError();
 }
 
@@ -264,6 +288,10 @@
   g.tiles_m = (M + WBM - 1) / WBM;
   g.tiles_n = (N + WBN - 1) / WBN;
   g.nt32 = bfrag_nt32(N);
+  if (batch.a_bias != nullptr) {
+    if (terms == 9) return launch_w8<9, true>(c, g);
+    return launch_w8<6, true>(c, g);
+  }
   if (terms == 9) return launch_w8<9>(c, g);
   return launch_w8<6>(c, g);
 }
diff --git a/relationprediction_amd/csrc/gemm_f32.hip b/relationprediction_amd/csrc/gemm_f32.hip
--- a/relationprediction_amd/csrc/gemm_f32.hip
+++ b/relationprediction_amd/csrc/gemm_f32.hip
@@ -311,11 +311,14 @@
   if (M <= 0 || N <= 0) return RGCN_OK;
   const int groups = batch ? batch->groups : 1;
   if (a_kc == false && b_kc == true) RGCN_FAIL(c, RGCN_ERR_UNSUPPORTED, "gemm TT form not instantiated");
+  if (batch && batch->a_bias != nullptr && (c->gemm_mode == 0 || !a_kc || b_kc || split_k > 1))
+    RGCN_FAIL(c, RGCN_ERR_UNSUPPORTED, "gemm: the A-operand prologue exists in the pre-split-weight NN kernels only");
   const int bk = 16;
   GemmArgs g;
   g.A = A; g.B = B; g.M = M; g.N = N; g.K = K; g.lda = lda; g.ldb = ldb;
-  const bool vec = vec_ok(A, lda, a_kc ? K : M) && vec_ok(B, ldb, b_kc ? K : N) &&
-                   (!batch || (batch->strideA % 4 == 0 && batch->strideB % 4 == 0));
+  const bool b_unread = batch && batch->bfrag != nullptr && a_kc && !b_kc && c->gemm_mode != 0 && split_k <= 1;
+  const bool vec = vec_ok(A, lda, a_kc ? K : M) && (b_unread || vec_ok(B, ldb, b_kc ? K : N)) &&
+                   (!batch || (batch->strideA % 4 == 0 && (b_unread || batch->strideB % 4 == 0)));
   g.swizzle = 1;
   g.zeros = c->zeros;
   if (batch) g.batch = *batch;
@@ -337,7 +340,8 @@
   }
   g.vecC = ((reinterpret_cast<uintptr_t>(g.C) & 15u) == 0 && g.ldc % 4 == 0 && N % 4 == 0) ? 1 : 0;
   {
-    ProfScope ps(c, tag, prof_scale * groups * 4.0 * ((double)M * K + (double)K * N + (double)M * N),
+    const double a_out_elems = batch && batch->a_bias && batch->a_out ? (double)M * K : 0.0;
+    ProfScope ps(c, tag, prof_scale * groups * 4.0 * ((double)M * K + (double)K * N + (double)M * N + a_out_elems),
                  prof_scale * groups * 2.0 * M * N * K);
     if (c->gemm_mode != 0) {
       RGCN_HIP(c, gemm_bf16x3_launch(c, c->gemm_mode, a_kc, b_kc, vec, M, N, K, A, lda, B, ldb, g.C, g.ldc,
diff --git a/relationprediction_amd/csrc/gemm_split.h b/relationprediction_amd/csrc/gemm_split.h
--- a/relationprediction_amd/csrc/gemm_split.h
+++ b/relationprediction_amd/csrc/gemm_split.h
@@ -39,6 +39,7 @@
 }
 
 constexpr int BM = 128, BN = 128, BK = 16, NTH = 256;
+constexpr int PRO_MAX_KT = 127;
 constexpr int KC_LD = 12;
 constexpr int RC_LD = 136;
 constexpr int KC_PLANE = 128 * KC_LD;
diff --git a/relationprediction_amd/csrc/rgcn_devtools.hip b/relationprediction_amd/csrc/rgcn_devtools.hip
--- a/relationprediction_amd/csrc/rgcn_devtools.hip
+++ b/relationprediction_amd/csrc/rgcn_devtools.hip
@@ -89,6 +89,58 @@
   return s;
 }
 
+rgcn_status rgcn_debug_gemm_prologue(rgcn_ctx* c, int32_t wide, int32_t prologue, int32_t M, int32_t N, int32_t K,
+                                     int32_t lda, int32_t row_limit, const float* a_host, const float* bias_host,
+                                     const float* b_host, float* a_out_host, float* c_host) {
+  RGCN_NEED(c);
+  if (M <= 0 || N <= 0 || K <= 0 || lda < K || row_limit > M || !a_host || !bias_host || !b_host || !a_out_host || !c_host)
+    RGCN_FAIL(c, RGCN_ERR_INVALID, "bad arguments");
+  float *A = nullptr, *B = nullptr, *C = nullptr, *bias = nullptr, *Aout = nullptr;
+  int32_t* lim = nullptr;
+  void* F = nullptr;
+  rgcn_status s = RGCN_OK;
+  const char* prev = getenv("RGCN_GEMM_W8");
+  const std::string saved = prev ? prev : "";
+  setenv("RGCN_GEMM_W8", wide ? "3" : "0", 1);
+  do {
+    if ((s = dmalloc(c, &A, (size_t)M * lda, false)) != RGCN_OK) break;
+    if ((s = dmalloc(c, &Aout, (size_t)M * lda, false)) != RGCN_OK) break;
+    if ((s = dmalloc(c, &B, (size_t)K * N, false)) != RGCN_OK) break;
+    if ((s = dmalloc(c, &bias, (size_t)K, false)) != RGCN_OK) break;
+    if ((s = dmalloc(c, &C, (size_t)M * N)) != RGCN_OK) break;
+    if ((s = dmalloc(c, &lim, 1)) != RGCN_OK) break;
+    if (hipMalloc(&F, 16 * gemm_bfrag_words(K, N)) != hipSuccess) { s = RGCN_ERR_NOMEM; break; }
+    if ((s = to_dev(c, A, a_host, sizeof(float) * (size_t)M * lda)) != RGCN_OK) break;
+    if ((s = to_dev(c, Aout, a_out_host, sizeof(float) * (size_t)M * lda)) != RGCN_OK) break;
+    if ((s = to_dev(c, B, b_host, sizeof(float) * (size_t)K * N)) != RGCN_OK) break;
+    if ((s = to_dev(c, bias, bias_host, sizeof(float) * (size_t)K)) != RGCN_OK) break;
+    if (row_limit >= 0 && (s = to_dev(c, lim, &row_limit, sizeof(int32_t))) != RGCN_OK) break;
+    const PresplitJob pj{B, F, N, K, N, 0};
+    if ((s = gemm_presplit_b(c, &pj, 1)) != RGCN_OK) break;
+    GemmBatch gb;
+    gb.bfrag = F;
+    gb.wide = wide ? 1 : 0;
+    if (row_limit >= 0) gb.limit = lim;
+    if (prologue) {
+      if (!gemm_a_prologue_ok(c, N, K, A, lda, B, N, F)) { c->err = "no prologue kernel takes this product"; s = RGCN_ERR_UNSUPPORTED; break; }
+      gb.a_bias = bias;
+      gb.a_out = Aout;
+    }
+    if ((s = gemm_f32(c, "debug_gemm", true, false, M, N, K, A, lda, B, N, C, N, 1, &gb)) != RGCN_OK) break;
+    if ((s = to_host(c, c_host, C, sizeof(float) * (size_t)M * N)) != RGCN_OK) break;
+    s = to_host(c, a_out_host, Aout, sizeof(float) * (size_t)M * lda);
+  } while (0);
+  if (prev) setenv("RGCN_GEMM_W8", saved.c_str(), 1); else unsetenv("RGCN_GEMM_W8");
+  if (A) (void)hipFree(A);
+  if (Aout) (void)hipFree(Aout);
+  if (B) (void)hipFree(B);
+  if (bias) (void)hipFree(bias);
+  if (C) (void)hipFree(C);
+  if (lim) (void)hipFree(lim);
+  if (F) (void)hipFree(F);
+  return s;
+}
+
 rgcn_status rgcn_debug_gemm_time(rgcn_ctx* c, int32_t ta, int32_t tb, int32_t M, int32_t N, int32_t K,
                                  int32_t split_k, int32_t iters, const float* a_host,
                                  const float* b_host, float* avg_ms) {
diff --git a/relationprediction_amd/csrc/rgcn_internal.h b/relationprediction_amd/csrc/rgcn_internal.h
--- a/relationprediction_amd/csrc/rgcn_internal.h
+++ b/relationprediction_amd/csrc/rgcn_internal.h
@@ -343,6 +343,7 @@
   bool frag_fresh = false;
   bool wtile_fresh = false;
   bool fwd_done = false;
+  bool h0_in_gemm = false;
   int fwd_train = 0;
   uint64_t seed = 0;
   bool explicit_masks = false;
@@ -425,8 +426,11 @@
   const void* bfrag = nullptr;
   size_t strideBfrag = 0;
   int wide = 0;
+  const float* a_bias = nullptr;
+  float* a_out = nullptr;
 };
 size_t gemm_bfrag_words(int K, int N);
+bool gemm_a_prologue_ok(const rgcn_ctx* c, int N, int K, const float* A, int lda, const float* B, int ldb, const void* bfrag);
 struct PresplitJob {
   const float* B;
   void* F;
diff --git a/relationprediction_amd/csrc/rgcn_schedule.hip b/relationprediction_amd/csrc/rgcn_schedule.hip
--- a/relationprediction_amd/csrc/rgcn_schedule.hip
+++ b/relationprediction_amd/csrc/rgcn_schedule.hip
@@ -1,6 +1,8 @@
 #include "rgcn_api_internal.h"
 
 namespace rgcn {
+
+static bool h0_by_self_loop_gemm(const rgcn_ctx* c);
 
 rgcn_status fwd_begin(rgcn_ctx* c, int train, uint64_t seed, const uint8_t* masks_host) {
   if (!c->g.ready) RGCN_FAIL(c, RGCN_ERR_STATE, "rgcn_forward before rgcn_set_graph");
@@ -18,6 +20,8 @@
     c->explicit_masks = true;
   }
   if (c->onehot) return RGCN_OK;
+  c->h0_in_gemm = h0_by_self_loop_gemm(c);
+  if (c->h0_in_gemm) return RGCN_OK;
   return input_forward(c);
 }
 
@@ -39,6 +43,13 @@
 }
 
 static bool rows_layer(const rgcn_ctx* c) { return c->fuse == 1 && block_rows_available(c); }
+
+constexpr int kH0InGemmDefault = 1;
+static bool h0_by_self_loop_gemm(const rgcn_ctx* c) {
+  if (knob("RGCN_H0_IN_GEMM", kH0InGemmDefault) == 0) return false;
+  if (c->onehot || c->world != 1 || c->kind != RGCN_KIND_BLOCK || !rows_layer(c) || c->L < 1) return false;
+  return gemm_a_prologue_ok(c, c->d, c->d, c->w_emb, c->d, c->layers[1].wself, c->d, c->layers[1].wself_nn);
+}
 
 static rgcn_status refresh_weight_fragments(rgcn_ctx* c) {
   if (c->gemm_mode == 0) return RGCN_OK;
@@ -91,6 +102,16 @@
   const double Mmsg = 2.0 * c->g.E / c->world;
   GemmBatch sb;
   RGCN_TRY(self_loop_batch(c, l, false, &sb));
+  if (l == 1 && c->h0_in_gemm) {
+    c->h0_in_gemm = false;
+    if (h0_by_self_loop_gemm(c)) {
+      Hin = c->w_emb;
+      sb.a_bias = c->b_emb;
+      sb.a_out = c->H[0];
+    } else {
+      RGCN_TRY(input_forward(c));
+    }
+  }
   if (c->kind == RGCN_KIND_BLOCK && rows_layer(c)) {
     RGCN_TRY(gemm_f32(c, "gemm_self_fwd", true, false, hi - lo, d, d, Hin + (size_t)lo * d, d, c->layers[l].wself, d,
                       c->self_buf + (size_t)lo * d, d, 1, &sb));
@@ -102,7 +123,7 @@
     a.row_lo = lo; a.row_hi = hi;
     a.drop = make_drop(c, l, true);
     a.drop2 = make_drop(c, l, false);
-    RGCN_TRY(block_rows(c, "block_rows_fwd", l, false, Hin, a));
+    RGCN_TRY(block_rows(c, "block_rows_fwd", l, false, c->H[l - 1], a));
   } else if (c->kind == RGCN_KIND_BLOCK) {
     {
       StreamScope side(c, 0);
```

Result: faster. 31.40 million edges/s, median of 6 (+1.6%).
